# yjxiong/action-detection

Measured on NVIDIA H100. Metric: proposals/sec (9-seg BNInception SSN fwd+bwd), higher is better.
Workload: dtype f32 via split f16 operands (hi+lo, 3 wgmma MMAs per product) / f32 accumulate; f32 storage

## Files before the change

### action-detection_b200/csrc/common.cuh

```cuda
#pragma once
#include <cuda_fp16.h>
#include <cuda_runtime.h>
#include <stdint.h>

#include <atomic>
#include <string>

namespace ssnb {

struct View {
  void* base = nullptr;
  int H = 0, W = 0, C = 0, pitch = 0, coff = 0;
  long long lo_off = 0;
};

extern std::atomic<long long> g_launches;
void set_thread_error(const std::string& s);
const std::string& thread_error();

struct LaunchTag {
  int phase = 3;
  double flop = 0.0;
  const char* op = nullptr;
  int tiles = 0, block_n = 0;
};
extern thread_local bool t_timing;
extern thread_local LaunchTag t_tag;
void timing_mark(const char* what, cudaStream_t s);

#define SSNB_LAUNCH_CHECK(what)                                                       \
  do {                                                                                \
    ssnb::g_launches.fetch_add(1, std::memory_order_relaxed);                         \
    cudaError_t _e = cudaGetLastError();                                              \
    if (_e != cudaSuccess) {                                                          \
      ssnb::set_thread_error(std::string(what) + ": " + cudaGetErrorString(_e));      \
      return 2;                                                                       \
    }                                                                                 \
    if (ssnb::t_timing) ssnb::timing_mark(what, s);                                   \
  } while (0)

template <typename T> __device__ __forceinline__ float to_f(T v);
template <> __device__ __forceinline__ float to_f<float>(float v) { return v; }
template <> __device__ __forceinline__ float to_f<__half>(__half v) { return __half2float(v); }
template <typename T> __device__ __forceinline__ T from_f(float v);
template <> __device__ __forceinline__ float from_f<float>(float v) { return v; }
template <> __device__ __forceinline__ __half from_f<__half>(float v) { return __float2half_rn(v); }
__device__ __forceinline__ float relu(float v) { return v <= 0.f ? 0.f : v; }

constexpr float HALF_MAX = 65504.f;
__device__ __forceinline__ void split2(float a, float b, uint32_t& hi, uint32_t& lo) {
  const __half2 h = __floats2half2_rn(a, b);
  const float2 hf = __half22float2(h);
  const __half2 l = __floats2half2_rn(a - hf.x, b - hf.y);
  hi = *reinterpret_cast<const uint32_t*>(&h);
  lo = *reinterpret_cast<const uint32_t*>(&l);
}
__device__ __forceinline__ void store_planes4(__half* hi, long long lo_off, const float4& v) {
  uint2 h, l;
  split2(v.x, v.y, h.x, l.x);
  split2(v.z, v.w, h.y, l.y);
  *reinterpret_cast<uint2*>(hi) = h;
  *reinterpret_cast<uint2*>(reinterpret_cast<char*>(hi) + lo_off) = l;
}

struct ConvArgs {
  const void* src; int SH, SW, Csrc, src_pitch, src_coff;
  void* dst;       int DH, DW, Cdst, dst_pitch, dst_coff;
  const void* wgt;
  const float* bias;
  int F, kh, kw, stride, pad_h, pad_w;
  int relu, accumulate, dgrad;
};
struct WgradArgs {
  const void* dz; int OH, OW, Cout, dz_pitch, dz_coff;
  const void* x;  int IH, IW, Cin, x_pitch, x_coff;
  float* partial;
  int F, k, stride, pad, rows_per_split, splits;
};
template <typename T> int launch_conv(const ConvArgs& a, cudaStream_t s);
template <typename T> int launch_wgrad(const WgradArgs& a, cudaStream_t s);
int launch_wgrad_finalize(const float* partial, int splits, int taps, int Cout, int Cin, const float* mult,
                          float out_scale, float* dw_ref, int accumulate, cudaStream_t s, const float* bias_partial = nullptr,
                          float* db = nullptr, int* flag = nullptr,
                          const float* unscale = nullptr);

template <typename T> int launch_nchw_to_nhwc(const float* src, int F, int C, int H, int W, View dst, float scale, cudaStream_t s);
template <typename T> int launch_nhwc_to_nchw(View src, int F, float scale, float* dst, cudaStream_t s);
template <typename T> int launch_gpool_fwd(View src, int F, float* feat, cudaStream_t s);
template <typename T> int launch_gpool_bwd(const float* dfeat, float scale, const float* scale_dev, View ddst, int F, const void* y,
                                           cudaStream_t s);
constexpr int GRAD_EXP_TOP = 8, GRAD_EXP_MAX = 100;
int launch_grad_exponent(const float* dfeat, long long n, float grad_scale, int HW, float* gscale, int* flag, cudaStream_t s);

constexpr int PACK_MAX = 32;
constexpr int PACK_PER_THREAD = 4;
constexpr int PACK_TILE = 32, PACK_TILE_TAPS = 9;
inline int pack_ctas(int cout, int cin, int taps) {
  if (taps <= PACK_TILE_TAPS) return ((cout + PACK_TILE - 1) / PACK_TILE) * ((cin + PACK_TILE - 1) / PACK_TILE);
  const long long n = (long long)cout * cin * taps, per = 256LL * PACK_PER_THREAD;
  return (int)(((n > cout ? n : cout) + per - 1) / per);
}
struct PackEntry {
  const float *w, *b, *gamma, *beta, *mean, *var;
  void *wf, *wd; float *bias, *scale, *absmax;
  int cout, cin, taps, block0;
  int nofold, pad_[3];
  float* bias_b;
};
struct PackTable { int n, pad_; PackEntry e[PACK_MAX]; };
template <typename T> int launch_pack_all(const PackTable& t, int total_blocks, cudaStream_t s);
struct SplitEntry {
  const float *wf, *wd; __half *wf16, *wd16; long long plane_bytes, n; const float* absmax; float* inv_scale; int block0, pad_;
  __half *wd16_b, *wf16_b; long long b_plane_bytes; int b_pitch, cout;
};
struct SplitTable { int n, pad_; SplitEntry e[PACK_MAX]; };
int launch_split_all(const SplitTable& t, int total_blocks, cudaStream_t s);

constexpr int FIN_MAX = 36;
struct FinalizeEntry {
  const float* partial; const float* mult; float* dw; const float* bias_partial; float* db;
  int splits, taps, Cout, Cin, block0, pad_;
};
struct FinalizeTable { int n, total_blocks; int* flag; const float* unscale; FinalizeEntry e[FIN_MAX]; };
int launch_wgrad_finalize_all(const FinalizeTable& t, float out_scale, int accumulate, cudaStream_t s);

template <typename T> constexpr int VEC_WIDTH = 16 / (int)sizeof(T);
template <typename T>
int launch_maxpool_fwd_vec(View src, View dst, View dst_planes, int F, int k, int stride, int pad, uint8_t* argmax, cudaStream_t s);
template <typename T>
int launch_maxpool_bwd_vec(View dsrc, View ddst, int F, int k, int stride, int pad, const uint8_t* argmax, int accumulate, cudaStream_t s);
template <typename T> int launch_avgpool3_vec(View src, View dst, View dst_planes, int F, int accumulate, cudaStream_t s);
template <typename T>
int launch_mask_bias_vec(View dy, View y, View planes, float scale, int write_back, int* flag, int F, const float* mult, float out_scale,
                         const float* unscale, float* partial, int max_ctas, float* db, int accumulate, cudaStream_t s);
template <typename T>
int launch_pool_mask_bias_vec(View dz, View y, View dpool, View planes, float scale, int write_back, int* flag, int F, int k, int stride, int pad,
                              const uint8_t* argmax, const float* mult, float out_scale, const float* unscale, float* partial, int max_ctas,
                              float* db, int accumulate, cudaStream_t s);
int launch_split_view(View src_f32, int F, float scale, View planes, int* flag, cudaStream_t s);
int launch_planes_to_nchw(View planes, int F, float scale, float* dst, cudaStream_t s);
int launch_bn_train_fwd(View z, View y, View y_planes, int F, const float* gamma, const float* beta, float eps, float momentum, float* running_mean,
                        float* running_var, float* stat, float* partial, int max_ctas, cudaStream_t s);
int launch_bn_train_bwd(View z, View dy, View y, View dz, View dz_planes, float plane_scale, int* flag, int F, const float* gamma, float* stat,
                        float* partial, int max_ctas, float* dgamma, float* dbeta, const float* unscale, int accumulate, cudaStream_t s);
int launch_nhwc_to_s2d(View src, int F, __half* dst, long long lo_off, int Cs, cudaStream_t s);
int launch_nchw_to_s2d(const float* src, int F, int Cin, int H, int W, __half* dst, long long lo_off, int Cs, cudaStream_t s);
int launch_pack_conv1_s2d(const __half* wd, int Cout, int Cin, int Cs, __half* ws, cudaStream_t s);
int launch_wgrad_finalize_s2d(const float* partial, int splits, int Cout, int Cin, int Cs, const float* mult, float out_scale,
                              const float* unscale, float* dw_ref, int accumulate, cudaStream_t s);
int launch_upsample2_zero(View src, __half* dst, int H, int W, int F, cudaStream_t s);

}
```

### action-detection_b200/csrc/engine.cu

```cuda
#include <cstdio>
#include <cstdlib>
#include <algorithm>
#include <cstring>
#include <map>
#include <string>
#include <vector>

#include <cuda_profiler_api.h>

#include "../../include/ssnb.h"
#include "common.cuh"
#include "graph.cuh"
#include "umma_conv.cuh"

namespace ssnb {

std::atomic<long long> g_launches{0};
static thread_local std::string t_error;
void set_thread_error(const std::string& s) { t_error = s; }
const std::string& thread_error() { return t_error; }

thread_local bool t_timing = false;
thread_local LaunchTag t_tag;
struct TimingMark { const char* what; LaunchTag tag; std::string op; cudaEvent_t ev; };
static thread_local std::vector<TimingMark> t_marks;
static thread_local std::vector<cudaEvent_t> t_event_pool;
static thread_local std::string t_report;
static cudaEvent_t timing_event() {
  if (!t_event_pool.empty()) { cudaEvent_t e = t_event_pool.back(); t_event_pool.pop_back(); return e; }
  cudaEvent_t e = nullptr;
  cudaEventCreate(&e);
  return e;
}
void timing_mark(const char* what, cudaStream_t s) {
  TimingMark m{what, t_tag, t_tag.op ? t_tag.op : "", timing_event()};
  m.tag.op = nullptr;
  if (m.ev && cudaEventRecord(m.ev, s) == cudaSuccess) t_marks.push_back(m);
  else cudaGetLastError();
  t_tag.flop = 0.0; t_tag.op = nullptr; t_tag.tiles = 0; t_tag.block_n = 0;
}

static bool timing_close() {
  t_timing = false;
  if (t_marks.empty()) return false;
  if (cudaEventSynchronize(t_marks.back().ev) != cudaSuccess) { cudaGetLastError(); return false; }
  return true;
}

struct BlockSpec { const char* name; int c1, c3r, c3, cdr, cd1, cd2; int pool_max; int cproj; int stride; };
static const BlockSpec kBlocks[10] = {
    {"3a", 64, 64, 64, 64, 96, 96, 0, 32, 1},      {"3b", 64, 64, 96, 64, 96, 96, 0, 64, 1},
    {"3c", 0, 128, 160, 64, 96, 96, 1, 0, 2},      {"4a", 224, 64, 96, 96, 128, 128, 0, 128, 1},
    {"4b", 192, 96, 128, 96, 128, 128, 0, 128, 1}, {"4c", 160, 128, 160, 128, 160, 160, 0, 128, 1},
    {"4d", 96, 128, 192, 160, 192, 192, 0, 128, 1}, {"4e", 0, 128, 192, 192, 256, 256, 1, 0, 2},
    {"5a", 352, 192, 320, 160, 224, 224, 0, 128, 1}, {"5b", 352, 192, 320, 192, 224, 224, 1, 128, 1}};

static std::vector<Conv> conv_table(int in_ch) {
  std::vector<Conv> v;
  auto add = [&](const std::string& id, int cin, int cout, int k, int stride, int pad) { v.push_back({id, cin, cout, k, k, stride, pad, pad}); };
  add("conv1_7x7_s2", in_ch, 64, 7, 2, 3);
  add("conv2_3x3_reduce", 64, 64, 1, 1, 0);
  add("conv2_3x3", 64, 192, 3, 1, 1);
  int cx = 192;
  for (const BlockSpec& b : kBlocks) {
    std::string p = std::string("inception_") + b.name + "_";
    if (b.c1) add(p + "1x1", cx, b.c1, 1, 1, 0);
    add(p + "3x3_reduce", cx, b.c3r, 1, 1, 0);
    add(p + "3x3", b.c3r, b.c3, 3, b.stride, 1);
    add(p + "double_3x3_reduce", cx, b.cdr, 1, 1, 0);
    add(p + "double_3x3_1", b.cdr, b.cd1, 3, 1, 1);
    add(p + "double_3x3_2", b.cd1, b.cd2, 3, b.stride, 1);
    if (b.cproj) add(p + "pool_proj", cx, b.cproj, 1, 1, 0);
    cx = b.c1 + b.c3 + b.cd2 + (b.cproj ? b.cproj : cx);
  }
  return v;
}

struct Op : GraphOp {
  int grad_accumulate = 0;
  int wsplits = 1, wrows = 0;
  int tsplits = 1;
  size_t partial_off = 0, bias_partial_off = 0;
  UmmaConvPlan umma;
  UmmaConvPlan umma_dgrad;
  UmmaWgradPlan umma_wgrad;
  int pool_consumer = -1;
  bool folded_into_conv = false;
  bool dgrad_masks = false;
  bool bias_in_wgrad = false;
  bool dy_premasked = false;
  bool raw = false;
  int fuse_role = 0;
  int fuse_block = -1;
};
struct FusedBlock {
  int op1 = -1, op_r3 = -1, op_rd = -1;
  int c1 = 0, c3r = 0, cdr = 0, cx = 0;
  size_t w_fwd = 0, bias = 0, w_dg = 0;
  size_t w_fwd_plane = 0, w_dg_plane = 0, wmax = 0;
  UmmaConvPlan fwd, dgrad;
  bool enabled = false;
};

}

using namespace ssnb;

struct ssnb_engine : ssnb::Graph<ssnb::Op> {
  ssnb_config cfg;
  size_t up_plane = 0, s2d_plane = 0, s2d_w_plane = 0;
  int* tc_flag = nullptr;
  size_t tc_flag_off = 0;
  float* gscale = nullptr;
  bool bn1_train = false;
  const float *bn1_gamma = nullptr, *bn1_beta = nullptr; float *bn1_rmean = nullptr, *bn1_rvar = nullptr, *bn1_dgamma = nullptr, *bn1_dbeta = nullptr;
  float bn1_momentum = 0.1f, bn1_eps = 1e-5f;
  size_t bn_stat_off = 0, bn_partial_off = 0;
  std::vector<FusedBlock> fused;
  size_t ws_bytes = 0, partial_off = 0, partial_bytes = 0, bpartial_off = 0;
  size_t s2d_off = 0, s2d_w_off = 0, up_off = 0;
  bool fold_pools = true;
  bool s2d_ready = false;
  int Cs = 0;
  int conv1_tsplits = 128;
  bool weights_ready = false;
  std::vector<float*> dw, db;
  std::vector<int> pending_finalize;
  int grad_accumulate = 0;
  std::string error;
  long long launches0 = 0;
  UmmaContext umma_ctx;

  int fail(int code, const std::string& msg) { error = msg; return code; }
  const float* grad_scale_dev() const { return tensor_cores() ? gscale : nullptr; }
  const float* grad_unscale_dev() const { return tensor_cores() ? gscale + 1 : nullptr; }
  int nplanes() const { return exact_tc() ? 2 : 1; }
  const __half* w_fwd(const PackedConv& p) const { return (const __half*)(ws + (exact_tc() ? p.wd16 : p.wd)); }
  const __half* w_dgrad(const PackedConv& p) const { return (const __half*)(ws + (exact_tc() ? p.wf16 : p.wf)); }
  const UmmaTcOpts* tc_opts(UmmaTcOpts& t, size_t w_lo_off, void* out32, float alpha, size_t wmax) const {
    if (!exact_tc()) return nullptr;
    t.w_lo_off = (long long)w_lo_off; t.out32 = (float*)out32; t.alpha = alpha; t.alpha_dev = (const float*)(ws + wmax) + 1;
    return &t;
  }
};

namespace ssnb {

static bool profiled_op(const char* env, const std::string& id) {
  const char* e = getenv(env);
  if (!e || !*e) return false;
  const std::string list = std::string(",") + e + ",";
  return list.find("," + id + ",") != std::string::npos;
}
static bool env_on(const char* name) {
  const char* v = getenv(name);
  return v && v[0] == '1';
}
static int device_sms() {
  int dev = 0, sms = 0;
  if (cudaGetDevice(&dev) != cudaSuccess || cudaDeviceGetAttribute(&sms, cudaDevAttrMultiProcessorCount, dev) != cudaSuccess || sms <= 0) {
    cudaGetLastError();
    return 132;
  }
  return sms;
}

static void build_graph(ssnb_engine* e) {
  const int cin = e->cfg.in_channels;
  e->convs = conv_table(cin);
  int ci = 0;
  auto conv_op = [&](int in, int out) {
    const Conv& c = e->convs[ci];
    Op o; o.kind = OP_CONV; o.id = c.id; o.in = in; o.out = out; o.conv = ci;
    o.k = c.kh; o.stride = c.stride; o.pad = c.ph;
    e->ops.push_back(o);
    ++ci;
  };
  auto pool_op = [&](OpKind kind, const std::string& id, int in, int out, int k, int s, int p) {
    Op o; o.kind = kind; o.id = id; o.in = in; o.out = out; o.k = k; o.stride = s; o.pad = p;
    e->ops.push_back(o);
  };
  int x = e->whole("data", 224, 224, cin);
  int v;
  if (e->bn1_train) {
    const int raw = e->whole("conv1_7x7_s2_raw", 112, 112, 64); conv_op(x, raw); e->ops.back().raw = true;
    v = e->whole("conv1_7x7_s2_bn", 112, 112, 64);
    pool_op(OP_BN1, "conv1_7x7_s2_bn", raw, v, 0, 1, 0); x = v;
  } else {
    v = e->whole("conv1_7x7_s2_bn", 112, 112, 64); conv_op(x, v); x = v;
  }
  v = e->whole("pool1_3x3_s2", 56, 56, 64); pool_op(OP_MAXPOOL, "pool1_3x3_s2", x, v, 3, 2, 0); x = v;
  v = e->whole("conv2_3x3_reduce_bn", 56, 56, 64); conv_op(x, v); x = v;
  v = e->whole("conv2_3x3_bn", 56, 56, 192); conv_op(x, v); x = v;
  v = e->whole("pool2_3x3_s2", 28, 28, 192); pool_op(OP_MAXPOOL, "pool2_3x3_s2", x, v, 3, 2, 0); x = v;
  int H = 28, cx = 192;
  for (const BlockSpec& b : kBlocks) {
    const std::string p = std::string("inception_") + b.name + "_";
    const int OHW = (b.stride == 2) ? pool_out(H, 3, 2, 0) : H;
    const int ctot = b.c1 + b.c3 + b.cd2 + (b.cproj ? b.cproj : cx);
    const int cat = e->add_buffer(p + "output", OHW, OHW, ctot);
    const int red = e->add_buffer(p + "reduce", H, H, b.c3r + b.cdr);
    int off = 0;
    if (b.c1) { v = e->add_value(p + "1x1_bn", cat, off, b.c1); conv_op(x, v); off += b.c1; }
    int r3 = e->add_value(p + "3x3_reduce_bn", red, 0, b.c3r); conv_op(x, r3);
    v = e->add_value(p + "3x3_bn", cat, off, b.c3); conv_op(r3, v); off += b.c3;
    int rd = e->add_value(p + "double_3x3_reduce_bn", red, b.c3r, b.cdr); conv_op(x, rd);
    int d1 = e->whole(p + "double_3x3_1_bn", H, H, b.cd1); conv_op(rd, d1);
    v = e->add_value(p + "double_3x3_2_bn", cat, off, b.cd2); conv_op(d1, v); off += b.cd2;
    if (b.stride == 2) {
      v = e->add_value(p + "pool", cat, off, cx);
      pool_op(OP_MAXPOOL, p + "pool", x, v, 3, 2, 0);
    } else {
      int pl = e->whole(p + "pool", H, H, cx);
      pool_op(b.pool_max ? OP_MAXPOOL : OP_AVGPOOL, p + "pool", x, pl, 3, 1, 1);
      v = e->add_value(p + "pool_proj_bn", cat, off, b.cproj); conv_op(pl, v);
    }
    x = e->add_value(p + "output", cat, 0, ctot);
    H = OHW; cx = ctot;
  }
  Op g; g.kind = OP_GPOOL; g.id = "global_pool"; g.in = x; g.out = -1; g.k = 7;
  e->ops.push_back(g);
}

static void plan(ssnb_engine* e) {
  const size_t F = (size_t)e->F;
  size_t off = 0;
  e->tc_flag_off = off; off = align_up(off + 256, 1024);
  if (e->bn1_train) { e->bn_stat_off = off; off = align_up(off + 4 * 64 * 4, 1024); e->bn_partial_off = off; off = align_up(off + (size_t)1200 * 2 * 64 * 4, 1024); }
  off = e->plan_storage(off, e->cfg.training != 0, e->convs[0].cin, 16);
  size_t pmax = 0;
  if (e->cfg.training) {
    std::vector<char> written(e->vals.size(), 0);
    for (int i = (int)e->ops.size() - 1; i >= 0; --i) {
      Op& o = e->ops[i];
      o.grad_accumulate = written[o.in];
      written[o.in] = 1;
      if (o.kind == OP_CONV) {
        const Conv& c = e->convs[o.conv];
        const Buffer& ob = e->bufs[e->vals[o.out].buf];
        const long long M = (long long)F * ob.H * ob.W;
        const int taps = c.kh * c.kw;
        const bool flat = c.cin < 16;
        const long long tiles = (long long)((c.cout + 63) / 64) * (flat ? (taps * c.cin + 63) / 64 : ((c.cin + 63) / 64) * taps);
        long long splits = (592 + tiles - 1) / tiles;
        if (splits > 128) splits = 128;
        while (splits > 1 && M / splits < 256) --splits;
        long long rows = (M + splits - 1) / splits;
        rows = (rows + 15) / 16 * 16;
        splits = (M + rows - 1) / rows;
        o.wsplits = (int)splits; o.wrows = (int)rows;
        {
          const int chunks = (c.cin + 63) / 64, n_tiles = (chunks + 3) / 4, block_n = ((chunks + n_tiles - 1) / n_tiles) * 64;
          const int tpc = std::max(1, 4 / (block_n / 64));
          const int ctas = ((c.cout + 127) / 128) * n_tiles * ((taps + tpc - 1) / tpc);
          o.tsplits = std::max(o.wsplits, std::min(128, umma_wgrad_splits(ctas, umma_wgrad_ptiles(ob.W, ob.H, e->F), device_sms())));
        }
        if (e->tensor_cores()) splits = std::max<long long>(splits, o.tsplits);
        const size_t need = (size_t)splits * taps * c.cout * c.cin * 4;
        if (need > pmax) pmax = need;
      }
    }
  }
  if (e->tensor_cores()) {
    for (int i = 0; i < (int)e->ops.size(); ++i) {
      const Op& o = e->ops[i];
      if (o.kind != OP_CONV || o.k != 1) continue;
      const std::string& id = o.id;
      const std::string suf = "_3x3_reduce";
      if (id.size() < suf.size() || id.compare(id.size() - suf.size(), suf.size(), suf) != 0 || id.find("double") != std::string::npos) continue;
      const std::string pre = id.substr(0, id.size() - suf.size() + 1);
      FusedBlock fb; fb.op_r3 = i;
      for (int j = 0; j < (int)e->ops.size(); ++j) {
        if (e->ops[j].id == pre + "1x1") fb.op1 = j;
        if (e->ops[j].id == pre + "double_3x3_reduce") fb.op_rd = j;
      }
      if (fb.op_rd < 0) continue;
      fb.cx = e->convs[o.conv].cin; fb.c3r = e->convs[o.conv].cout; fb.cdr = e->convs[e->ops[fb.op_rd].conv].cout;
      fb.c1 = fb.op1 >= 0 ? e->convs[e->ops[fb.op1].conv].cout : 0;
      const int n = fb.c1 + fb.c3r + fb.cdr, kf = (fb.c1 + 63) / 64 * 64 + fb.c3r + fb.cdr;
      fb.w_fwd_plane = align_up((size_t)n * fb.cx * 2, 1024); fb.w_dg_plane = align_up((size_t)fb.cx * kf * 2, 1024);
      if (e->exact_tc()) fb.w_fwd_plane = fb.w_dg_plane = std::max(fb.w_fwd_plane, fb.w_dg_plane);
      fb.w_fwd = off; off += e->nplanes() * fb.w_fwd_plane;
      fb.bias = off; off = align_up(off + (size_t)n * 4, 256);
      fb.w_dg = off; off += e->nplanes() * fb.w_dg_plane;
      if (e->exact_tc()) {
        if (e->fused.size() >= 16) continue;
        fb.wmax = e->wmax_off + (e->convs.size() + e->fused.size()) * 8;
        for (int j : {fb.op1, fb.op_r3, fb.op_rd}) if (j >= 0) e->packed[e->ops[j].conv].wmax = fb.wmax;
      }
      e->fused.push_back(fb);
    }
  }
  if (e->tensor_cores()) {
    for (int i = 0; i < (int)e->ops.size(); ++i) {
      Op& po = e->ops[i];
      if (po.kind != OP_MAXPOOL || po.k != 3 || po.stride != 2 || po.pad != 0) continue;
      int producer = -1, consumers = 0;
      for (int j = 0; j < (int)e->ops.size(); ++j) {
        if (e->ops[j].out == po.in && e->ops[j].kind == OP_CONV) producer = j;
        if (e->ops[j].in == po.in) ++consumers;
      }
      if (producer >= 0 && consumers == 1 && e->vals[po.in].C % (e->fast() ? VEC_WIDTH<__half> : VEC_WIDTH<float>) == 0) { e->ops[producer].pool_consumer = i; po.folded_into_conv = true; }
    }
    auto operand_region = [&](size_t bytes, size_t& plane) {
      const size_t at = off;
      if (e->exact_tc()) { plane = align_up(bytes, 1024); off += 2 * plane; }
      else off = align_up(off + bytes, 1024);
      return at;
    };
    e->Cs = (4 * e->cfg.in_channels + 7) / 8 * 8;
    {
      const int chunks = (4 * e->Cs + 63) / 64, n_tiles = (chunks + 3) / 4, block_n = ((chunks + n_tiles - 1) / n_tiles) * 64;
      const int tpc = std::min(4, std::max(1, 4 / (block_n / 64)));
      const int ptiles = umma_wgrad_ptiles(112, 112, e->F);
      if ((ptiles + UMMA_WGRAD_MAX_PTILES - 1) / UMMA_WGRAD_MAX_PTILES > 128)
        e->conv1_tsplits = umma_wgrad_splits(n_tiles * ((4 + tpc - 1) / tpc), ptiles, device_sms());
    }
    e->s2d_off = operand_region(F * 112 * 112 * 4 * e->Cs * 2, e->s2d_plane);
    e->s2d_w_off = operand_region((size_t)16 * 64 * e->Cs * 2, e->s2d_w_plane);
    if (e->cfg.training) {
      size_t up = 0;
      for (const Op& o : e->ops)
        if (o.kind == OP_CONV && o.stride == 2 && o.conv != 0) {
          const Buffer& ib = e->bufs[e->vals[o.in].buf];
          up = std::max(up, F * ib.H * ib.W * (size_t)e->convs[o.conv].cout * 2);
        }
      e->up_off = operand_region(up, e->up_plane);
      pmax = std::max(pmax, (size_t)e->conv1_tsplits * 16 * 64 * e->Cs * 4);
    }
  }
  e->partial_off = off; e->partial_bytes = pmax; off = align_up(off + pmax, 1024);
  if (e->cfg.training)
    for (Op& o : e->ops)
      if (o.kind == OP_CONV) {
        const Conv& c = e->convs[o.conv];
        const int nsplit = e->tensor_cores() ? std::max(o.wsplits, o.tsplits) : o.wsplits;
        size_t need = (size_t)nsplit * c.kh * c.kw * c.cout * c.cin * 4;
        if (o.conv == 0 && e->tensor_cores()) need = std::max(need, (size_t)e->conv1_tsplits * 16 * 64 * e->Cs * 4);
        o.partial_off = off; off = align_up(off + need, 1024);
        o.bias_partial_off = off; off = align_up(off + (size_t)std::max(nsplit, 128) * c.cout * 4, 256);
      }
  e->bpartial_off = off; off = align_up(off + (size_t)1024 * 512 * 4, 1024);
  e->ws_bytes = off;
}

#define DISPATCH(e, call_f, call_h) ((e)->fast() ? (call_h) : (call_f))

static inline void tag_next(int phase, double flop, const char* op = nullptr) { t_tag.phase = phase; t_tag.flop = flop; t_tag.op = op; }
static thread_local std::string t_fused_name;
static const char* fused_name(const ssnb_engine* e, const FusedBlock& fb) {
  if (!t_timing) return nullptr;
  t_fused_name.clear();
  for (int j : {fb.op1, fb.op_r3, fb.op_rd})
    if (j >= 0) t_fused_name += (t_fused_name.empty() ? "" : "+") + e->ops[j].id;
  return t_fused_name.c_str();
}

static int run_fwd(ssnb_engine* e, const Op& o, float* feat, int n, cudaStream_t s) {
  tag_next(0, 0.0);
  if (o.kind == OP_CONV && o.umma.enabled) {
    if (o.conv == 0 && !e->s2d_ready) {
      const View in = e->view(o.in, false);
      __half* s2d = (__half*)(e->ws + e->s2d_off);
      if (int rc = launch_nhwc_to_s2d(in, n, s2d, (long long)e->s2d_plane, e->Cs, s)) return rc;
    }
    tag_next(0, e->conv_flops(o, n), o.id.c_str());
    return umma_conv_launch(e->umma_ctx, o.umma, s, false, n);
  }
  if (o.kind == OP_BN1) {
    if (!e->bn1_gamma || !e->bn1_beta) { set_thread_error("bn1_train engine: call ssnb_set_bn1 first"); return SSNB_ESTATE; }
    return launch_bn_train_fwd(e->view(o.in, false), e->view(o.out, false), e->exact_tc() ? e->planes(o.out, false) : View(), e->F, e->bn1_gamma,
                               e->bn1_beta, e->bn1_eps, e->bn1_momentum, e->bn1_rmean, e->bn1_rvar, (float*)(e->ws + e->bn_stat_off),
                               (float*)(e->ws + e->bn_partial_off), 1200, s);
  }
  if (o.kind == OP_MAXPOOL || o.kind == OP_AVGPOOL) return e->pool_fwd(o, n, s);
  if (o.kind == OP_GPOOL) {
    if (!feat) return e->fail(SSNB_EINVAL, "global_pool needs the feat output pointer");
    return e->gpool_fwd(o, n, feat, s);
  }
  if (int rc = e->simt_conv_fwd(o, o.raw ? 0 : 1, n, s)) return rc;
  if (!e->exact_tc() || !e->bufs[e->vals[o.out].buf].plane) return 0;
  return launch_split_view(e->view(o.out), n, 1.0f, e->planes(o.out), nullptr, s);
}

static int simt_wgrad(ssnb_engine* e, const Op& o, cudaStream_t s) {
  const Conv& c = e->convs[o.conv];
  const View x = e->view(o.in, false), dz = e->view(o.out, true);
  float* partial = (float*)(e->ws + o.partial_off);
  WgradArgs w;
  w.dz = dz.base; w.OH = dz.H; w.OW = dz.W; w.Cout = dz.C; w.dz_pitch = dz.pitch; w.dz_coff = dz.coff;
  w.x = x.base; w.IH = x.H; w.IW = x.W; w.Cin = x.C; w.x_pitch = x.pitch; w.x_coff = x.coff;
  w.partial = partial; w.F = e->F; w.k = c.kh; w.stride = c.stride; w.pad = c.ph;
  w.rows_per_split = o.wrows; w.splits = o.wsplits;
  tag_next(2, e->conv_flops(o, e->F), o.id.c_str());
  if (int rc = DISPATCH(e, launch_wgrad<float>(w, s), launch_wgrad<__half>(w, s))) return rc;
  const float out_scale = e->fast() ? 1.0f / e->cfg.grad_scale : 1.0f;
  return launch_wgrad_finalize(partial, o.wsplits, c.kh * c.kw, c.cout, c.cin, (const float*)(e->ws + e->packed[o.conv].scale), out_scale,
                               e->dw[o.conv], e->grad_accumulate, s, nullptr, nullptr, nullptr, e->grad_unscale_dev());
}
static int simt_dgrad(ssnb_engine* e, const Op& o, cudaStream_t s) {
  const Conv& c = e->convs[o.conv];
  const View dz = e->view(o.out, true), dx = e->view(o.in, true);
  ConvArgs a;
  a.src = dz.base; a.SH = dz.H; a.SW = dz.W; a.Csrc = dz.C; a.src_pitch = dz.pitch; a.src_coff = dz.coff;
  a.dst = dx.base; a.DH = dx.H; a.DW = dx.W; a.Cdst = dx.C; a.dst_pitch = dx.pitch; a.dst_coff = dx.coff;
  a.wgt = e->ws + e->packed[o.conv].wd; a.bias = nullptr;
  a.F = e->F; a.kh = a.kw = c.kh; a.stride = c.stride; a.pad_h = a.pad_w = c.ph; a.relu = 0; a.accumulate = o.grad_accumulate; a.dgrad = 1;
  tag_next(1, e->conv_flops(o, e->F), o.id.c_str());
  return DISPATCH(e, launch_conv<float>(a, s), launch_conv<__half>(a, s));
}

static int run_bwd(ssnb_engine* e, const Op& o, const float* dfeat, cudaStream_t s, bool skip_dgrad = false, bool full = false) {
  const int F = e->F;
  const float gs = e->fast() ? e->cfg.grad_scale : 1.0f;
  int rc = 0;
  tag_next(3, 0.0);
  if (o.kind == OP_GPOOL) {
    if (!dfeat) return e->fail(SSNB_EINVAL, "global_pool backward needs dfeat");
    const View din = e->view(o.in, true);
    const void* ym = (full && e->fold_pools && o.dgrad_masks) ? e->view(o.in, false).base : nullptr;
    const float* gsd = e->grad_scale_dev();
    return DISPATCH(e, launch_gpool_bwd<float>(dfeat, gs, gsd, din, F, ym, s), launch_gpool_bwd<__half>(dfeat, gs, gsd, din, F, ym, s));
  }
  if (o.kind == OP_BN1) {
    return launch_bn_train_bwd(e->view(o.in, false), e->view(o.out, true), e->view(o.out, false), e->view(o.in, true),
                               e->exact_tc() ? e->planes(o.in, true) : View(), e->cfg.grad_scale, e->tc_flag, F, e->bn1_gamma, (float*)(e->ws + e->bn_stat_off),
                               (float*)(e->ws + e->bn_partial_off), 1200, e->bn1_dgamma, e->bn1_dbeta, e->grad_unscale_dev(), e->grad_accumulate, s);
  }
  if (o.kind == OP_MAXPOOL) {
    if (full && e->fold_pools && o.folded_into_conv) return 0;
    const View din = e->view(o.in, true), dout = e->view(o.out, true);
    const uint8_t* am = (const uint8_t*)(e->ws + o.argmax_off);
    return DISPATCH(e, launch_maxpool_bwd_vec<float>(din, dout, F, o.k, o.stride, o.pad, am, o.grad_accumulate, s),
                    launch_maxpool_bwd_vec<__half>(din, dout, F, o.k, o.stride, o.pad, am, o.grad_accumulate, s));
  }
  if (o.kind == OP_AVGPOOL) {
    const View din = e->view(o.in, true), dout = e->view(o.out, true);
    return DISPATCH(e, launch_avgpool3_vec<float>(dout, din, View(), F, o.grad_accumulate, s),
                    launch_avgpool3_vec<__half>(dout, din, View(), F, o.grad_accumulate, s));
  }
  const Conv& c = e->convs[o.conv];
  const View x = e->view(o.in, false), y = e->view(o.out, false), dy = e->view(o.out, true);
  const float* scale = (const float*)(e->ws + e->packed[o.conv].scale);
  float* bpartial = (float*)(e->ws + e->bpartial_off);
  float* dbp = (e->db.size() && e->db[o.conv]) ? e->db[o.conv] : nullptr;
  const bool want_w = e->dw.size() && e->dw[o.conv];
  const bool want_x = e->vals[o.in].name != "data" && !skip_dgrad;
  const float gst = e->cfg.grad_scale;
  const float* us = e->grad_unscale_dev();
  const bool tc_w = want_w && o.umma_wgrad.enabled, tc_x = want_x && o.umma_dgrad.enabled;
  const bool pre = full && e->fold_pools && o.dy_premasked;
  const bool bias_w = pre && o.bias_in_wgrad && dbp && tc_w;
  const Op* pool = (full && e->fold_pools && o.pool_consumer >= 0) ? &e->ops[o.pool_consumer] : nullptr;
  const int max_ctas = (1024 * 512 - 64) / y.C;
  const View dpool = pool ? e->view(pool->out, true) : View();
  const uint8_t* pam = pool ? (const uint8_t*)(e->ws + pool->argmax_off) : nullptr;
  if (e->fast()) {
    if (pool) rc = launch_pool_mask_bias_vec<__half>(dy, y, dpool, View(), 1.0f, 1, nullptr, F, pool->k, pool->stride, pool->pad, pam,
                                                    scale, 1.0f / gst, us, bpartial, max_ctas, dbp, e->grad_accumulate, s);
    else if (!bias_w) rc = launch_mask_bias_vec<__half>(dy, pre ? View() : y, View(), 1.0f, 1, nullptr, F, scale, 1.0f / gst, us, bpartial, max_ctas, dbp,
                                                       e->grad_accumulate, s);
  } else {
    const bool need_f32 = (want_w && !tc_w) || (want_x && !tc_x);
    const View pl = (tc_w || tc_x) ? e->planes(o.out, true) : View();
    if (o.raw) {
      if (dbp) rc = launch_mask_bias_vec<float>(dy, View(), View(), gst, 0, nullptr, F, scale, 1.0f, us, bpartial, max_ctas, dbp, e->grad_accumulate, s);
    } else if (pre) {
      if (!bias_w && dbp) rc = launch_mask_bias_vec<float>(dy, y, View(), gst, 0, nullptr, F, scale, 1.0f, us, bpartial, max_ctas, dbp, e->grad_accumulate, s);
    } else if (pool) {
      rc = launch_pool_mask_bias_vec<float>(dy, y, dpool, pl, gst, need_f32 ? 1 : 0, e->tc_flag, F, pool->k, pool->stride, pool->pad, pam,
                                            scale, 1.0f, us, bpartial, max_ctas, dbp, e->grad_accumulate, s);
    } else {
      rc = launch_mask_bias_vec<float>(dy, y, pl, gst, (need_f32 || !full) ? 1 : 0, e->tc_flag, F, scale, 1.0f, us, bpartial, max_ctas, dbp,
                                       e->grad_accumulate, s);
    }
  }
  if (rc) return rc;
  if (tc_x && c.stride == 2 && o.conv != 0) {
    View dz = e->operand(o.out, true);
    for (int p = 0; p < e->nplanes(); ++p, dz.base = (char*)dz.base + dz.lo_off)
      if ((rc = launch_upsample2_zero(dz, (__half*)(e->ws + e->up_off + p * e->up_plane), x.H, x.W, F, s))) return rc;
  }
  if (tc_w) {
    float* partial = (float*)(e->ws + o.partial_off);
    float* bp = bias_w ? (float*)(e->ws + o.bias_partial_off) : nullptr;
    tag_next(2, e->conv_flops(o, F), o.id.c_str());
    if ((rc = umma_wgrad_launch(e->umma_ctx, o.umma_wgrad, s, bp))) return rc;
    if (full && o.conv != 0) e->pending_finalize.push_back((int)(&o - e->ops.data()));
    else if (o.conv == 0) rc = launch_wgrad_finalize_s2d(partial, o.umma_wgrad.p.splits, c.cout, c.cin, e->Cs, scale, 1.0f / gst, us, e->dw[o.conv],
                                                         e->grad_accumulate, s);
    else rc = launch_wgrad_finalize(partial, o.umma_wgrad.p.splits, c.kh * c.kw, c.cout, c.cin, scale, 1.0f / gst, e->dw[o.conv], e->grad_accumulate, s,
                                    nullptr, nullptr, e->tc_flag, us);
    if (rc) return rc;
  } else if (want_w && (rc = simt_wgrad(e, o, s))) return rc;
  if (tc_x) {
    tag_next(1, e->conv_flops(o, F), o.id.c_str());
    return umma_conv_launch(e->umma_ctx, o.umma_dgrad, s, full && e->fold_pools && o.dgrad_masks);
  }
  return want_x ? simt_dgrad(e, o, s) : 0;
}

int engine_tail_view(ssnb_handle h, View* v, int* F, int* fp16) {
  if (!h->ws || !h->weights_ready) return h->fail(SSNB_ESTATE, "workspace/weights not set");
  *v = h->view(h->ops.back().in, false);
  *F = h->F; *fp16 = h->fast() ? 1 : 0;
  return 0;
}

}

extern "C" {

const char* ssnb_version(void) { return "libssn_b200 0.3 (sm_90a)"; }

const char* ssnb_last_error(ssnb_handle h) { return h ? h->error.c_str() : ssnb::thread_error().c_str(); }

int ssnb_num_convs(void) { return 69; }

int ssnb_conv_info(int idx, int in_channels, char* name, int name_cap, int* cin, int* cout, int* k, int* stride, int* pad) {
  std::vector<Conv> t = conv_table(in_channels);
  if (idx < 0 || idx >= (int)t.size()) { set_thread_error("ssnb_conv_info: index out of range"); return SSNB_EINVAL; }
  if (name && name_cap > 0) { snprintf(name, name_cap, "%s", t[idx].id.c_str()); }
  if (cin) *cin = t[idx].cin; if (cout) *cout = t[idx].cout; if (k) *k = t[idx].kh;
  if (stride) *stride = t[idx].stride; if (pad) *pad = t[idx].ph;
  return SSNB_OK;
}

int ssnb_create(const ssnb_config* cfg, ssnb_handle* out) {
  if (!cfg || !out) { set_thread_error("ssnb_create: null argument"); return SSNB_EINVAL; }
  if (cfg->frames <= 0 || cfg->in_channels <= 0 || cfg->in_channels > 64) { set_thread_error("ssnb_create: bad frames/in_channels"); return SSNB_EINVAL; }
  if (cfg->precision != SSNB_EXACT_FP32 && cfg->precision != SSNB_FAST_FP16 && cfg->precision != SSNB_EXACT_TC) { set_thread_error("ssnb_create: unknown precision"); return SSNB_EINVAL; }
  ssnb_engine* e = new ssnb_engine();
  e->cfg = *cfg;
  if (!(e->cfg.grad_scale > 0.f)) e->cfg.grad_scale = 1.0f;
  e->F = cfg->frames;
  e->precision = cfg->precision;
  e->bn1_train = cfg->bn1_train != 0;
  if (e->bn1_train && e->fast()) { delete e; set_thread_error("ssnb_create: bn1_train (bn_mode='partial') needs EXACT_FP32 or EXACT_TC"); return SSNB_ENOSUPPORT; }
  e->esz = e->fast() ? 2 : 4;
  build_graph(e);
  if ((int)e->convs.size() != 69) { delete e; set_thread_error("internal: conv table size"); return SSNB_ESTATE; }
  umma_context_init(e->umma_ctx);
  plan(e);
  e->launches0 = g_launches.load();
  *out = e;
  return SSNB_OK;
}

int ssnb_destroy(ssnb_handle h) {
  if (!h) return SSNB_OK;
  umma_context_destroy(h->umma_ctx);
  delete h;
  return SSNB_OK;
}

size_t ssnb_workspace_bytes(ssnb_handle h) { return h ? h->ws_bytes : 0; }

int ssnb_set_workspace(ssnb_handle h, void* dev_ptr, size_t bytes) {
  if (!h) return SSNB_EINVAL;
  if (!dev_ptr || bytes < h->ws_bytes) return h->fail(SSNB_EINVAL, "workspace too small");
  if (((uintptr_t)dev_ptr) % 1024) return h->fail(SSNB_EINVAL, "workspace must be 1024-byte aligned");
  h->ws = (char*)dev_ptr;
  h->weights_ready = false;
  if (cudaMemset(h->ws + h->bpartial_off, 0, 256) != cudaSuccess) { cudaGetLastError();  }
  h->tc_flag = (int*)(h->ws + h->tc_flag_off);
  if (cudaMemset(h->tc_flag, 0, 256) != cudaSuccess) cudaGetLastError();
  h->gscale = (float*)(h->ws + h->tc_flag_off + 16);
  const float one[2] = {1.0f, 1.0f};
  if (cudaMemcpy(h->gscale, one, sizeof one, cudaMemcpyHostToDevice) != cudaSuccess) cudaGetLastError();
  const bool training = h->cfg.training != 0;
  const bool use_tc = h->tensor_cores() && !env_on("SSNB_DISABLE_UMMA");
  const bool use_wgrad = use_tc && training && !env_on("SSNB_DISABLE_UMMA_WGRAD");
  const bool fuse = !env_on("SSNB_DISABLE_FUSION");
  const float gs = h->cfg.grad_scale;
  for (Op& o : h->ops) {
    o.umma.enabled = o.umma_dgrad.enabled = o.umma_wgrad.enabled = false;
    o.fuse_role = 0; o.fuse_block = -1; o.dgrad_masks = o.dy_premasked = o.bias_in_wgrad = false;
  }
  for (FusedBlock& fb : h->fused) fb.enabled = false;
  h->fold_pools = fuse && (h->fast() || (use_tc && training));
  auto tc_gate = [&](UmmaConvPlan& p) {
    if (h->exact_tc() && !p.p.tc_ok) p.enabled = false;
    return p.enabled;
  };
  for (Op& o : h->ops) {
    if (o.kind != OP_CONV || !use_tc) continue;
    const Conv& c = h->convs[o.conv];
    const PackedConv& pk = h->packed[o.conv];
    UmmaTcOpts tf, tg;
    int rc = 0;
    if (o.conv == 0) {
      const int Ck = 4 * h->Cs;
      View xs; xs.base = h->ws + h->s2d_off; xs.H = 112; xs.W = 112; xs.C = Ck; xs.pitch = Ck; xs.coff = 0; xs.lo_off = (long long)h->s2d_plane;
      int dy[4], dx[4];
      for (int t = 0; t < 4; ++t) { dy[t] = t - 2; dx[t] = 0; }
      rc = umma_conv_bind_taps(h->umma_ctx, o.umma, xs, h->operand(o.out, false), h->F, Ck, c.cout, 4, dy, dx, (const __half*)(h->ws + h->s2d_w_off),
                               (const float*)(h->ws + pk.bias), o.raw ? 0 : 1, h->tc_opts(tf, h->s2d_w_plane, h->view(o.out, false).base, 1.0f, pk.wmax));
      if (rc) return h->fail(rc, "conv1 bind: " + ssnb::thread_error());
      tc_gate(o.umma);
      if (use_wgrad && (rc = umma_wgrad_bind_taps(h->umma_ctx, o.umma_wgrad, h->operand(o.out, true), xs, h->F, Ck, c.cout, 4, dy, dx,
                                                  (float*)(h->ws + o.partial_off), h->conv1_tsplits)))
        return h->fail(rc, "conv1 wgrad bind: " + ssnb::thread_error());
      continue;
    }
    if (c.cin % 8 != 0 || c.kh * c.kw > UMMA_MAX_TAPS) continue;
    rc = umma_conv_bind_fwd(h->umma_ctx, o.umma, h->operand(o.in, false), h->operand(o.out, false), h->F, c.cin, c.cout, c.kh, c.ph,
                            c.stride, h->w_fwd(pk), (const float*)(h->ws + pk.bias), h->tc_opts(tf, pk.wplane, h->view(o.out, false).base, 1.0f, pk.wmax));
    if (rc) return h->fail(rc, "bind_fwd(" + c.id + "): " + ssnb::thread_error());
    if (!training) continue;
    const View in = h->view(o.in, false);
    View dz = h->operand(o.out, true);
    if (c.stride == 2) { dz.base = h->ws + h->up_off; dz.H = in.H; dz.W = in.W; dz.C = c.cout; dz.pitch = c.cout; dz.coff = 0; dz.lo_off = (long long)h->up_plane; }
    View dx = h->view(o.in, true);
    const UmmaTcOpts* og = h->tc_opts(tg, pk.wplane, dx.base, 1.0f / gs, pk.wmax);
    if (og) dx.base = nullptr;
    rc = umma_conv_bind_dgrad(h->umma_ctx, o.umma_dgrad, dz, dx, h->F, c.cin, c.cout, c.kh, c.ph, h->w_dgrad(pk), o.grad_accumulate, og);
    if (rc) return h->fail(rc, "bind_dgrad(" + c.id + "): " + ssnb::thread_error());
    tc_gate(o.umma_dgrad);
    if (use_wgrad && (rc = umma_wgrad_bind(h->umma_ctx, o.umma_wgrad, h->operand(o.out, true), h->operand(o.in, false), h->F, c.cin, c.cout,
                                           c.kh, c.ph, (float*)(h->ws + o.partial_off), o.tsplits, c.stride)))
      return h->fail(rc, "wgrad_bind(" + c.id + "): " + ssnb::thread_error());
  }
  for (size_t bi = 0; bi < h->fused.size() && use_tc && fuse; ++bi) {
    FusedBlock& fb = h->fused[bi];
    const Op& o3 = h->ops[fb.op_r3]; const Op& od = h->ops[fb.op_rd];
    if (!o3.umma.enabled || !od.umma.enabled) continue;
    const int nr = fb.c3r + fb.cdr;
    const View x = h->operand(o3.in, false);
    View red = h->operand(o3.out, false); red.C = nr;
    UmmaTcOpts tf, tg;
    int rc;
    if (fb.op1 >= 0) {
      const int v1 = h->ops[fb.op1].out;
      const UmmaTcOpts* of = h->tc_opts(tf, fb.w_fwd_plane, h->view(v1, false).base, 1.0f, fb.wmax);
      tf.out32_2 = (float*)h->view(o3.out, false).base;
      rc = umma_conv_bind_fused_fwd(h->umma_ctx, fb.fwd, x, h->operand(v1, false), red, h->F, fb.cx, fb.c1, nr, (const __half*)(h->ws + fb.w_fwd),
                                    (const float*)(h->ws + fb.bias), of);
    } else {
      rc = umma_conv_bind_fwd(h->umma_ctx, fb.fwd, x, red, h->F, fb.cx, nr, 1, 0, 1, (const __half*)(h->ws + fb.w_fwd), (const float*)(h->ws + fb.bias),
                              h->tc_opts(tf, fb.w_fwd_plane, h->view(o3.out, false).base, 1.0f, fb.wmax));
    }
    if (rc) return h->fail(rc, "fused fwd bind(" + o3.id + "): " + ssnb::thread_error());
    if (!tc_gate(fb.fwd)) continue;
    if (training) {
      View dred = h->operand(o3.out, true); dred.C = nr;
      const View d1 = fb.op1 >= 0 ? h->operand(h->ops[fb.op1].out, true) : dred;
      View dx = h->view(o3.in, true);
      const UmmaTcOpts* og = h->tc_opts(tg, fb.w_dg_plane, dx.base, 1.0f / gs, fb.wmax);
      if (og) dx.base = nullptr;
      rc = umma_conv_bind_fused_dgrad(h->umma_ctx, fb.dgrad, d1, dred, dx, h->F, fb.cx, fb.c1, nr, (const __half*)(h->ws + fb.w_dg), od.grad_accumulate, og);
      if (rc) return h->fail(rc, "fused dgrad bind(" + o3.id + "): " + ssnb::thread_error());
      if (!tc_gate(fb.dgrad)) continue;
      if (h->exact_tc() && cudaMemset(h->ws + fb.w_dg, 0, 2 * fb.w_dg_plane) != cudaSuccess) cudaGetLastError();
    }
    fb.enabled = true;
    const int leader = fb.op1 >= 0 ? fb.op1 : fb.op_r3;
    for (int j : {fb.op1, fb.op_r3, fb.op_rd})
      if (j >= 0) { h->ops[j].fuse_block = (int)bi; h->ops[j].fuse_role = (j == leader) ? 1 : 2; }
  }
  if (use_tc && training && fuse) {
    std::vector<int> first_consumer(h->vals.size(), -1);
    for (int i = 0; i < (int)h->ops.size(); ++i)
      if (first_consumer[h->ops[i].in] < 0) first_consumer[h->ops[i].in] = i;
    for (size_t v = 0; v < h->vals.size(); ++v) {
      const int fc = first_consumer[v];
      if (fc < 0 || h->vals[v].name == "data") continue;
      if (h->exact_tc() && !h->bufs[h->vals[v].buf].plane) continue;
      bool conv_made = false;
      for (const Op& q : h->ops) conv_made = conv_made || (q.kind == OP_CONV && h->vals[q.out].buf == h->vals[v].buf);
      if (!conv_made) continue;
      Op& c = h->ops[fc];
      UmmaConvPlan* dg = nullptr;
      if (c.kind == OP_CONV && c.fuse_role == 1 && h->fused[c.fuse_block].enabled) dg = &h->fused[c.fuse_block].dgrad;
      else if (c.kind == OP_CONV && c.fuse_role == 0 && c.umma_dgrad.enabled) dg = &c.umma_dgrad;
      if (dg) {
        c.dgrad_masks = true;
        if (h->exact_tc()) {
          if (int rc = umma_conv_set_mask_tc(h->umma_ctx, *dg, h->view((int)v, false), h->planes((int)v, true), gs, h->tc_flag))
            return h->fail(rc, "mask bind(" + h->vals[v].name + "): " + ssnb::thread_error());
        } else {
          umma_conv_set_mask(*dg, h->view((int)v, false));
        }
      } else if (c.kind == OP_GPOOL && h->fast()) {
        c.dgrad_masks = true;
      }
    }
    for (Op& o : h->ops) {
      if (o.kind != OP_CONV) continue;
      int w = o.out;
      if (first_consumer[w] < 0) {
        const Value& ov = h->vals[o.out];
        for (size_t v = 0; v < h->vals.size(); ++v)
          if (h->vals[v].buf == ov.buf && h->vals[v].coff == 0 && h->vals[v].C == h->bufs[ov.buf].C && first_consumer[v] >= 0) { w = (int)v; break; }
      }
      if (first_consumer[w] >= 0 && h->ops[first_consumer[w]].dgrad_masks) o.dy_premasked = true;
      o.bias_in_wgrad = o.dy_premasked && o.conv != 0 && o.umma_wgrad.enabled;
    }
  }
  return SSNB_OK;
}

int ssnb_pack_weights(ssnb_handle h, const float* const* w, const float* const* b, const float* const* gamma,
                      const float* const* beta, const float* const* mean, const float* const* var, void* stream) {
  if (!h || !h->ws) return h ? h->fail(SSNB_ESTATE, "set_workspace first") : SSNB_EINVAL;
  cudaStream_t s = (cudaStream_t)stream;
  struct Member { int block = -1, row = 0, col = 0; };
  std::vector<Member> member(h->convs.size());
  for (size_t bi = 0; bi < h->fused.size(); ++bi) {
    const FusedBlock& fb = h->fused[bi];
    if (!fb.enabled) continue;
    const int k1p = (fb.c1 + 63) / 64 * 64;
    int row = 0, col = 0;
    for (int j : {fb.op1, fb.op_r3, fb.op_rd}) {
      if (j < 0) continue;
      const int ci = h->ops[j].conv;
      member[ci].block = (int)bi; member[ci].row = row; member[ci].col = col;
      row += h->convs[ci].cout;
      col += (j == fb.op1) ? k1p : h->convs[ci].cout;
    }
  }
  auto adjust = [&](size_t i, PackEntry& q, SplitEntry* e) {
    q.nofold = (h->bn1_train && i == 0) ? 1 : 0;
    const Member& mb = member[i];
    if (!h->exact_tc() || mb.block < 0) return;
    const FusedBlock& fb = h->fused[mb.block];
    q.bias_b = (float*)(h->ws + fb.bias) + mb.row;
    const int kf = (fb.c1 + 63) / 64 * 64 + fb.c3r + fb.cdr;
    e->wd16_b = (__half*)(h->ws + fb.w_fwd) + (size_t)mb.row * fb.cx;
    e->wf16_b = (__half*)(h->ws + fb.w_dg) + mb.col;
    e->b_pitch = kf;
    e->b_plane_bytes = (long long)std::max(fb.w_fwd_plane, fb.w_dg_plane);
  };
  if (int rc = h->pack_weights(w, b, gamma, beta, mean, var, h->convs[0].cin, adjust, "pack_weights", s)) return h->fail(rc, ssnb::thread_error());
  if (h->ops.size() && h->ops[0].umma.enabled) {
    const PackedConv& p = h->packed[0];
    for (int pl = 0; pl < h->nplanes(); ++pl) {
      int rc = launch_pack_conv1_s2d((const __half*)((const char*)h->w_fwd(p) + pl * p.wplane), h->convs[0].cout, h->convs[0].cin, h->Cs,
                                     (__half*)(h->ws + h->s2d_w_off + pl * h->s2d_w_plane), s);
      if (rc) return h->fail(rc, "pack conv1 s2d: " + ssnb::thread_error());
    }
  }
  for (FusedBlock& fb : h->fused) {
    if (!fb.enabled || !h->fast()) continue;
    const int k1p = (fb.c1 + 63) / 64 * 64, kf = k1p + fb.c3r + fb.cdr;
    __half* wfwd = (__half*)(h->ws + fb.w_fwd); float* bias = (float*)(h->ws + fb.bias); __half* wdg = (__half*)(h->ws + fb.w_dg);
    if (cudaMemsetAsync(wdg, 0, (size_t)fb.cx * kf * 2, s) != cudaSuccess) return h->fail(SSNB_ECUDA, "fused pack: memset");
    int row = 0, col = 0;
    for (int j : {fb.op1, fb.op_r3, fb.op_rd}) {
      if (j < 0) { continue; }
      const int ci = h->ops[j].conv, co = h->convs[ci].cout;
      cudaError_t e1 = cudaMemcpyAsync(wfwd + (size_t)row * fb.cx, h->ws + h->packed[ci].wd, (size_t)co * fb.cx * 2, cudaMemcpyDeviceToDevice, s);
      cudaError_t e2 = cudaMemcpyAsync(bias + row, h->ws + h->packed[ci].bias, (size_t)co * 4, cudaMemcpyDeviceToDevice, s);
      cudaError_t e3 = cudaMemcpy2DAsync(wdg + col, (size_t)kf * 2, h->ws + h->packed[ci].wf, (size_t)co * 2, (size_t)co * 2, fb.cx,
                                         cudaMemcpyDeviceToDevice, s);
      if (e1 != cudaSuccess || e2 != cudaSuccess || e3 != cudaSuccess) return h->fail(SSNB_ECUDA, "fused pack: copy failed");
      row += co;
      col += (j == fb.op1) ? k1p : co;
    }
  }
  h->weights_ready = true;
  return SSNB_OK;
}

int ssnb_set_bn1(ssnb_handle h, const float* gamma, const float* beta, float* running_mean, float* running_var, float* dgamma, float* dbeta,
                 float momentum, float eps) {
  if (!h) return SSNB_EINVAL;
  if (!h->bn1_train) return h->fail(SSNB_ESTATE, "engine created without bn1_train");
  if (!gamma || !beta) return h->fail(SSNB_EINVAL, "set_bn1: gamma / beta are required");
  h->bn1_gamma = gamma; h->bn1_beta = beta; h->bn1_rmean = running_mean; h->bn1_rvar = running_var; h->bn1_dgamma = dgamma; h->bn1_dbeta = dbeta;
  h->bn1_momentum = momentum; h->bn1_eps = eps;
  return SSNB_OK;
}

static int backbone_fwd(ssnb_handle h, const float* input_nchw, int n, float* feat, cudaStream_t s) {
  const View d = h->view(h->val_by_name["data"], false);
  int rc;
  h->s2d_ready = h->tensor_cores() && h->ops[0].umma.enabled;
  if (h->s2d_ready) rc = launch_nchw_to_s2d(input_nchw, n, d.C, d.H, d.W, (__half*)(h->ws + h->s2d_off), (long long)h->s2d_plane, h->Cs, s);
  else rc = h->value_write(h->val_by_name["data"], false, input_nchw, 1.0f, n, s);
  if (rc) { h->s2d_ready = false; return h->fail(rc, "input layout: " + ssnb::thread_error()); }
  for (size_t i = 0; i < h->ops.size(); ++i) {
    const Op& o = h->ops[i];
    if (o.fuse_role == 2) continue;
    const bool prof = profiled_op("SSNB_PROFILE_FWD_OPS", o.id);
    if (prof) cudaProfilerStart();
    int r;
    if (o.fuse_role == 1) {
      const FusedBlock& fb = h->fused[o.fuse_block];
      double fl = 0.0;
      for (int j : {fb.op1, fb.op_r3, fb.op_rd}) if (j >= 0) fl += h->conv_flops(h->ops[j], n);
      tag_next(0, fl, fused_name(h, fb));
      r = umma_conv_launch(h->umma_ctx, fb.fwd, s, false, n);
    } else r = run_fwd(h, o, feat, n, s);
    if (prof) cudaProfilerStop();
    if (r) { h->s2d_ready = false; return h->fail(r, "fwd " + o.id + ": " + ssnb::thread_error()); }
  }
  h->s2d_ready = false;
  return SSNB_OK;
}

int ssnb_backbone_fwd(ssnb_handle h, const float* input_nchw, float* feat, void* stream) {
  if (!h || !input_nchw || !feat) return h ? h->fail(SSNB_EINVAL, "null argument") : SSNB_EINVAL;
  if (!h->ws || !h->weights_ready) return h->fail(SSNB_ESTATE, "workspace/weights not set");
  return backbone_fwd(h, input_nchw, h->F, feat, (cudaStream_t)stream);
}

int ssnb_backbone_fwd_frames(ssnb_handle h, const float* input_nchw, int frames, float* feat, void* stream) {
  if (!h || !input_nchw || !feat) return h ? h->fail(SSNB_EINVAL, "null argument") : SSNB_EINVAL;
  if (frames < 1 || frames > h->F) return h->fail(SSNB_EINVAL, "backbone_fwd_frames: frames must be in 1 .. " + std::to_string(h->F));
  if (h->cfg.training) return h->fail(SSNB_ESTATE, "backbone_fwd_frames: runs forward-only engines (training = 0)");
  if (h->bn1_train) return h->fail(SSNB_ENOSUPPORT, "backbone_fwd_frames: bn1_train engines run their planned frame count only");
  if (!h->ws || !h->weights_ready) return h->fail(SSNB_ESTATE, "workspace/weights not set");
  return backbone_fwd(h, input_nchw, frames, feat, (cudaStream_t)stream);
}

int ssnb_bind_grads(ssnb_handle h, float* const* dw, float* const* db) {
  if (!h) return SSNB_EINVAL;
  h->dw.assign(h->convs.size(), nullptr); h->db.assign(h->convs.size(), nullptr);
  for (size_t i = 0; i < h->convs.size(); ++i) { if (dw) h->dw[i] = dw[i]; if (db) h->db[i] = db[i]; }
  return SSNB_OK;
}

int ssnb_backbone_bwd(ssnb_handle h, const float* dfeat, float* const* dw, float* const* db, void* stream) {
  return ssnb_backbone_bwd_range(h, dfeat, dw, db, -1, 0, stream);
}

int ssnb_backbone_bwd_range(ssnb_handle h, const float* dfeat, float* const* dw, float* const* db, int op_hi, int op_lo, void* stream) {
  if (!h || (!dfeat && (op_hi < 0 || op_hi >= (int)h->ops.size() - 1))) return h ? h->fail(SSNB_EINVAL, "null argument") : SSNB_EINVAL;
  if (!h->cfg.training) return h->fail(SSNB_ESTATE, "engine created without training=1");
  if (!h->ws || !h->weights_ready) return h->fail(SSNB_ESTATE, "workspace/weights not set");
  ssnb_bind_grads(h, dw, db);
  h->pending_finalize.clear();
  cudaStream_t s = (cudaStream_t)stream;
  auto run_range = [&](int hi, int lo) -> int {
    for (int i = hi; i >= lo; --i) {
      const Op& o = h->ops[i];
      const bool prof = profiled_op("SSNB_PROFILE_BWD_OPS", o.id);
      if (prof) cudaProfilerStart();
      int rc = run_bwd(h, o, dfeat, s, o.fuse_role != 0, true);
      if (!rc && o.fuse_role == 1) {
        const FusedBlock& fb = h->fused[o.fuse_block];
        double fl = 0.0;
        for (int j : {fb.op1, fb.op_r3, fb.op_rd}) if (j >= 0) fl += h->conv_flops(h->ops[j], h->F);
        tag_next(1, fl, fused_name(h, fb));
        rc = umma_conv_launch(h->umma_ctx, fb.dgrad, s, h->fold_pools && o.dgrad_masks);
      }
      if (prof) cudaProfilerStop();
      if (rc) return h->fail(rc, "bwd " + o.id + ": " + ssnb::thread_error());
    }
    return 0;
  };
  auto finalize = [&]() -> int {
    const float gs = h->tensor_cores() ? h->cfg.grad_scale : 1.0f;
    FinalizeTable t; t.n = 0; t.total_blocks = 0; t.flag = h->tc_flag; t.unscale = h->grad_unscale_dev();
    auto flush = [&]() -> int { int rc = launch_wgrad_finalize_all(t, 1.0f / gs, h->grad_accumulate, s); t.n = 0; t.total_blocks = 0; return rc; };
    for (int oi : h->pending_finalize) {
      const Op& o = h->ops[oi];
      const Conv& c = h->convs[o.conv];
      FinalizeEntry& q = t.e[t.n];
      q.partial = (const float*)(h->ws + o.partial_off); q.mult = (const float*)(h->ws + h->packed[o.conv].scale); q.dw = h->dw[o.conv];
      const bool bias_w = o.dy_premasked && o.bias_in_wgrad && h->db.size() && h->db[o.conv];
      q.bias_partial = bias_w ? (const float*)(h->ws + o.bias_partial_off) : nullptr; q.db = bias_w ? h->db[o.conv] : nullptr;
      q.splits = o.umma_wgrad.p.splits; q.taps = c.kh * c.kw; q.Cout = c.cout; q.Cin = c.cin; q.block0 = t.total_blocks; q.pad_ = 0;
      t.total_blocks += (int)(((long long)q.taps * q.Cout * q.Cin + 255) / 256);
      if (++t.n == FIN_MAX) if (int rc = flush()) { h->pending_finalize.clear(); return h->fail(rc, "finalize: " + ssnb::thread_error()); }
    }
    h->pending_finalize.clear();
    if (int rc = flush()) return h->fail(rc, "finalize: " + ssnb::thread_error());
    return 0;
  };
  const int last = (int)h->ops.size() - 1;
  if (op_hi < 0 || op_hi > last) op_hi = last;
  if (op_lo < 0 || op_lo > op_hi) return h->fail(SSNB_EINVAL, "backbone_bwd_range: bad op range");
  if (op_hi == last && h->tensor_cores()) {
    if (int rc = launch_grad_exponent(dfeat, (long long)h->F * h->vals[h->ops[last].in].C, h->cfg.grad_scale,
                                      h->bufs[h->vals[h->ops[last].in].buf].H * h->bufs[h->vals[h->ops[last].in].buf].W, h->gscale, h->tc_flag, s))
      return h->fail(rc, "gradient exponent: " + ssnb::thread_error());
  }
  if (int rc = run_range(op_hi, op_lo)) return rc;
  return finalize();
}

int ssnb_set_grad_accumulate(ssnb_handle h, int accumulate) {
  if (!h) return SSNB_EINVAL;
  h->grad_accumulate = accumulate ? 1 : 0;
  return SSNB_OK;
}

int ssnb_num_ops(ssnb_handle h) { return h ? (int)h->ops.size() : 0; }

int ssnb_op_info(ssnb_handle h, int op, char* kind, int kind_cap, char* in_name, int in_cap, char* out_name, int out_cap) {
  if (!h || op < 0 || op >= (int)h->ops.size()) return SSNB_EINVAL;
  const Op& o = h->ops[op];
  if (kind) snprintf(kind, kind_cap, "%s", kOpKindName[o.kind]);
  if (in_name) snprintf(in_name, in_cap, "%s", h->vals[o.in].name.c_str());
  if (out_name) snprintf(out_name, out_cap, "%s", o.out >= 0 ? h->vals[o.out].name.c_str() : "feat");
  return SSNB_OK;
}

int ssnb_value_shape(ssnb_handle h, const char* name, int* c, int* hh, int* ww) {
  if (!h || !name) return SSNB_EINVAL;
  const int v = h->value_of(name);
  if (v < 0) return h->fail(SSNB_EINVAL, std::string("unknown value ") + name);
  const View w = h->view(v, false);
  if (c) *c = w.C; if (hh) *hh = w.H; if (ww) *ww = w.W;
  return SSNB_OK;
}

static float host_gscale(ssnb_handle h, int which, cudaStream_t s) {
  float v = 1.0f;
  if (!h->tensor_cores() || cudaMemcpyAsync(&v, h->gscale + which, sizeof v, cudaMemcpyDeviceToHost, s) != cudaSuccess ||
      cudaStreamSynchronize(s) != cudaSuccess) { cudaGetLastError(); return 1.0f; }
  return v;
}

int ssnb_value_write(ssnb_handle h, const char* name, int grad, const float* src_nchw, void* stream) {
  if (!h || !name || !src_nchw || !h->ws) return SSNB_EINVAL;
  const int v = h->value_of(name);
  if (v < 0) return h->fail(SSNB_EINVAL, std::string("unknown value ") + name);
  if (grad && !h->cfg.training) return h->fail(SSNB_ESTATE, "no gradient buffers");
  const float sc = grad ? (h->fast() ? h->cfg.grad_scale : 1.0f) * host_gscale(h, 0, (cudaStream_t)stream) : 1.0f;
  const int rc = h->value_write(v, grad != 0, src_nchw, sc, h->F, (cudaStream_t)stream);
  return rc ? h->fail(rc, ssnb::thread_error()) : SSNB_OK;
}

int ssnb_value_read(ssnb_handle h, const char* name, int grad, float* dst_nchw, void* stream) {
  if (!h || !name || !dst_nchw || !h->ws) return SSNB_EINVAL;
  const int v = h->value_of(name);
  if (v < 0) return h->fail(SSNB_EINVAL, std::string("unknown value ") + name);
  if ((grad & 1) && !h->cfg.training) return h->fail(SSNB_ESTATE, "no gradient buffers");
  if (grad & 2) {
    if (!h->exact_tc() || !h->bufs[h->vals[v].buf].plane) return h->fail(SSNB_ESTATE, "value has no operand planes");
    const float sc = (grad & 1) ? host_gscale(h, 1, (cudaStream_t)stream) / h->cfg.grad_scale : 1.0f;
    const int rc = h->planes_read(v, (grad & 1) != 0, sc, dst_nchw, (cudaStream_t)stream);
    return rc ? h->fail(rc, ssnb::thread_error()) : SSNB_OK;
  }
  const float sc = grad ? host_gscale(h, 1, (cudaStream_t)stream) / (h->fast() ? h->cfg.grad_scale : 1.0f) : 1.0f;
  const int rc = h->value_read(v, grad != 0, sc, dst_nchw, (cudaStream_t)stream);
  return rc ? h->fail(rc, ssnb::thread_error()) : SSNB_OK;
}

int ssnb_run_op(ssnb_handle h, int op, int backward, void* stream) {
  if (!h || op < 0 || op >= (int)h->ops.size()) return SSNB_EINVAL;
  if (!h->ws || !h->weights_ready) return h->fail(SSNB_ESTATE, "workspace/weights not set");
  const Op& o = h->ops[op];
  if (o.kind == OP_GPOOL) return h->fail(SSNB_ENOSUPPORT, "run_op: global_pool runs through backbone_fwd/bwd");
  int rc = backward ? run_bwd(h, o, nullptr, (cudaStream_t)stream) : run_fwd(h, o, nullptr, h->F, (cudaStream_t)stream);
  return rc ? h->fail(rc, o.id + ": " + ssnb::thread_error()) : SSNB_OK;
}

int ssnb_grad_overflow(ssnb_handle h, int clear) {
  if (!h) return -1;
  if (!h->tc_flag) return 0;
  int v = 0;
  if (cudaMemcpy(&v, h->tc_flag, sizeof(int), cudaMemcpyDeviceToHost) != cudaSuccess) { cudaGetLastError(); return -1; }
  if (v && clear) cudaMemset(h->tc_flag, 0, sizeof(int));
  return v ? 1 : 0;
}

int ssnb_timing_begin(void* stream) {
  for (TimingMark& m : ssnb::t_marks) ssnb::t_event_pool.push_back(m.ev);
  ssnb::t_marks.clear();
  ssnb::t_tag = LaunchTag();
  ssnb::t_timing = true;
  ssnb::timing_mark("(begin)", (cudaStream_t)stream);
  return SSNB_OK;
}

const char* ssnb_timing_report(void) {
  ssnb::t_report.clear();
  if (!ssnb::timing_close()) return ssnb::t_report.c_str();
  struct Agg { int n = 0; double ms = 0, flop = 0; };
  std::map<std::pair<std::string, int>, Agg> agg;
  for (size_t i = 1; i < ssnb::t_marks.size(); ++i) {
    float ms = 0.f;
    if (cudaEventElapsedTime(&ms, ssnb::t_marks[i - 1].ev, ssnb::t_marks[i].ev) != cudaSuccess) { cudaGetLastError(); continue; }
    Agg& a = agg[{ssnb::t_marks[i].what, ssnb::t_marks[i].tag.phase}];
    a.n += 1; a.ms += ms; a.flop += ssnb::t_marks[i].tag.flop;
  }
  char line[256];
  for (const auto& kv : agg) {
    snprintf(line, sizeof line, "%s\t%d\t%d\t%.6f\t%.0f\n", kv.first.first.c_str(), kv.first.second, kv.second.n, kv.second.ms, kv.second.flop);
    ssnb::t_report += line;
  }
  return ssnb::t_report.c_str();
}

const char* ssnb_timing_launches(void) {
  ssnb::t_report.clear();
  if (!ssnb::timing_close()) return ssnb::t_report.c_str();
  char line[512];
  for (size_t i = 1; i < ssnb::t_marks.size(); ++i) {
    const ssnb::TimingMark& m = ssnb::t_marks[i];
    float ms = 0.f;
    if (cudaEventElapsedTime(&ms, ssnb::t_marks[i - 1].ev, m.ev) != cudaSuccess) { cudaGetLastError(); continue; }
    snprintf(line, sizeof line, "%s\t%d\t%s\t%.6f\t%.0f\t%d\t%d\n", m.what, m.tag.phase, m.op.empty() ? "-" : m.op.c_str(), ms, m.tag.flop,
             m.tag.tiles, m.tag.block_n);
    ssnb::t_report += line;
  }
  return ssnb::t_report.c_str();
}

int64_t ssnb_launch_count(ssnb_handle h) { return h ? (int64_t)(g_launches.load() - h->launches0) : 0; }
int64_t ssnb_global_launch_count(void) { return (int64_t)g_launches.load(); }

}
```

### action-detection_b200/csrc/s2d_glue.cu

```cuda
#include "common.cuh"

#include <type_traits>

namespace ssnb {
namespace {

template <typename T>
__global__ void nhwc_to_s2d_kernel(const T* __restrict__ src, int F, int H, int W, int Cin, int spitch, int scoff,
                                   __half* __restrict__ dst, long long lo_off, int Cs) {
  const int H2 = H / 2, W2 = W / 2, Ck = 4 * Cs;
  const long long total = (long long)F * H2 * W2 * Ck;
  const long long i = (long long)blockIdx.x * blockDim.x + threadIdx.x;
  if (i >= total) return;
  const int ch = (int)(i % Ck);
  const long long p = i / Ck;
  const int x2 = (int)(p % W2), y2 = (int)((p / W2) % H2);
  const long long f = p / ((long long)W2 * H2);
  const int ds = ch / Cs, q = ch % Cs;
  T v = 0.f;
  const int xs = x2 + ds - 2;
  if (q < 4 * Cin && xs >= 0 && xs < W2) {
    const int ab = q / Cin, c = q % Cin;
    v = src[((f * H + 2 * y2 + ab / 2) * W + 2 * xs + ab % 2) * spitch + scoff + c];
  }
  if constexpr (std::is_same_v<T, float>) {
    const __half h = __float2half_rn(v);
    dst[i] = h;
    *reinterpret_cast<__half*>(reinterpret_cast<char*>(dst + i) + lo_off) = __float2half_rn(v - __half2float(h));
  } else {
    dst[i] = v;
  }
}

__global__ void pack_conv1_s2d_kernel(const __half* __restrict__ wd, int Cout, int Cin, int Cs, __half* __restrict__ ws) {
  const int Ck = 4 * Cs;
  const long long total = (long long)4 * Cout * Ck;
  const long long i = (long long)blockIdx.x * blockDim.x + threadIdx.x;
  if (i >= total) return;
  const int ch = (int)(i % Ck);
  const int co = (int)((i / Ck) % Cout);
  const int dr = (int)(i / ((long long)Ck * Cout));
  const int ds = ch / Cs, q = ch % Cs;
  __half v = __float2half_rn(0.f);
  if (q < 4 * Cin) {
    const int ab = q / Cin, c = q % Cin;
    const int r = 2 * dr + ab / 2 - 1, s = 2 * ds + ab % 2 - 1;
    if (r >= 0 && r < 7 && s >= 0 && s < 7) v = wd[((long long)(r * 7 + s) * Cout + co) * Cin + c];
  }
  ws[i] = v;
}

__global__ void wgrad_finalize_s2d_kernel(const float* __restrict__ partial, int splits, int Cout, int Cin, int Cs,
                                          const float* __restrict__ mult, float out_scale, const float* __restrict__ unscale,
                                          float* __restrict__ dw, int accumulate) {
  const int Ck = 4 * Cs;
  const long long total = (long long)Cout * Cin * 49;
  const long long i = (long long)blockIdx.x * blockDim.x + threadIdx.x;
  if (i >= total) return;
  const int s = (int)(i % 7), r = (int)((i / 7) % 7);
  const int c = (int)((i / 49) % Cin), co = (int)(i / (49LL * Cin));
  const int dr = (r + 1) / 2, a = (r + 1) % 2, ds = (s + 1) / 2, b = (s + 1) % 2;
  const int ch = ds * Cs + (a * 2 + b) * Cin + c;
  float acc = 0.f;
  for (int sp = 0; sp < splits; ++sp) acc += partial[(((long long)sp * 4 + dr) * Cout + co) * Ck + ch];
  if (unscale) out_scale *= __ldg(unscale);
  dw[i] = (accumulate ? dw[i] : 0.f) + acc * mult[co] * out_scale;
}

template <int CS, int CIN, bool LO>
__global__ void nchw_to_s2d_kernel(const float* __restrict__ src, int F, int Cin_rt, int H, int W, __half* __restrict__ dst,
                                   long long lo_off) {
  const int Cin = CIN ? CIN : Cin_rt;
  const int H2 = H / 2, W2 = W / 2;
  const long long i = (long long)blockIdx.x * blockDim.x + threadIdx.x;
  if (i >= (long long)F * H2 * W2 * 4) return;
  const unsigned iu = (unsigned)i;
  const int ds = (int)(iu & 3u);
  const unsigned pu = iu >> 2;
  const int x2 = (int)(pu % (unsigned)W2), y2 = (int)((pu / (unsigned)W2) % (unsigned)H2);
  const long long p = pu;
  const long long f = pu / (unsigned)(W2 * H2);
  __align__(16) __half vh[CS];
  __align__(16) __half vl[LO ? CS : 1];
#pragma unroll
  for (int c = 0; c < CS; ++c) {
    vh[c] = __float2half_rn(0.f);
    if constexpr (LO) vl[c] = __float2half_rn(0.f);
  }
  const int xs = x2 + ds - 2;
  if (xs >= 0 && xs < W2) {
#pragma unroll
    for (int c = 0; c < Cin; ++c) {
      const float* pl = src + ((f * Cin + c) * H + 2 * y2) * (long long)W + 2 * xs;
      const float2 r0 = __ldg(reinterpret_cast<const float2*>(pl));
      const float2 r1 = __ldg(reinterpret_cast<const float2*>(pl + W));
      const float q[4] = {r0.x, r0.y, r1.x, r1.y};
#pragma unroll
      for (int ab = 0; ab < 4; ++ab) {
        const __half h = __float2half_rn(q[ab]);
        vh[ab * Cin + c] = h;
        if constexpr (LO) vl[ab * Cin + c] = __float2half_rn(q[ab] - __half2float(h));
      }
    }
  }
  __half* o = dst + p * (4 * CS) + ds * CS;
  uint4* oh = reinterpret_cast<uint4*>(o);
  uint4* ol = reinterpret_cast<uint4*>(reinterpret_cast<char*>(o) + lo_off);
#pragma unroll
  for (int q = 0; q < CS / 8; ++q) {
    oh[q] = reinterpret_cast<const uint4*>(vh)[q];
    if constexpr (LO) ol[q] = reinterpret_cast<const uint4*>(vl)[q];
  }
}

__global__ void upsample2_zero_kernel(const __half* __restrict__ src, int OH, int OW, int C, int spitch, int scoff,
                                      __half* __restrict__ dst, int H, int W, int F) {
  const int G = C / 8;
  const long long total = (long long)F * H * W * G;
  const long long i = (long long)blockIdx.x * blockDim.x + threadIdx.x;
  if (i >= total) return;
  const unsigned iu = (unsigned)i;
  const int g = (int)(iu % (unsigned)G);
  const unsigned pu = iu / (unsigned)G;
  const int x = (int)(pu % (unsigned)W), y = (int)((pu / (unsigned)W) % (unsigned)H);
  const long long p = pu;
  const long long f = pu / (unsigned)(W * H);
  uint4 v = make_uint4(0u, 0u, 0u, 0u);
  if (!(x & 1) && !(y & 1) && y / 2 < OH && x / 2 < OW)
    v = __ldg(reinterpret_cast<const uint4*>(src + ((f * OH + y / 2) * OW + x / 2) * spitch + scoff + g * 8));
  *reinterpret_cast<uint4*>(dst + p * C + g * 8) = v;
}

}

int launch_nhwc_to_s2d(View src, int F, __half* dst, long long lo_off, int Cs, cudaStream_t s) {
  const long long n = (long long)F * (src.H / 2) * (src.W / 2) * 4 * Cs;
  const unsigned g = (unsigned)((n + 255) / 256);
  if (lo_off) nhwc_to_s2d_kernel<float><<<g, 256, 0, s>>>((const float*)src.base, F, src.H, src.W, src.C, src.pitch, src.coff, dst, lo_off, Cs);
  else nhwc_to_s2d_kernel<__half><<<g, 256, 0, s>>>((const __half*)src.base, F, src.H, src.W, src.C, src.pitch, src.coff, dst, lo_off, Cs);
  SSNB_LAUNCH_CHECK("nhwc_to_s2d_kernel");
  return 0;
}
template <bool LO>
static int nchw_to_s2d(const float* src, int F, int Cin, int H, int W, __half* dst, long long lo_off, int Cs, cudaStream_t s) {
  const long long n = (long long)F * (H / 2) * (W / 2) * 4;
  const unsigned g = (unsigned)((n + 255) / 256);
  if (Cs == 16 && Cin == 3) nchw_to_s2d_kernel<16, 3, LO><<<g, 256, 0, s>>>(src, F, Cin, H, W, dst, lo_off);
  else if (Cs == 40 && Cin == 10) nchw_to_s2d_kernel<40, 10, LO><<<g, 256, 0, s>>>(src, F, Cin, H, W, dst, lo_off);
  else if (Cs == 16) nchw_to_s2d_kernel<16, 0, LO><<<g, 256, 0, s>>>(src, F, Cin, H, W, dst, lo_off);
  else if (Cs == 40) nchw_to_s2d_kernel<40, 0, LO><<<g, 256, 0, s>>>(src, F, Cin, H, W, dst, lo_off);
  else { set_thread_error("nchw_to_s2d: unsupported channel count (RGB 3 or Flow 10)"); return 1; }
  SSNB_LAUNCH_CHECK("nchw_to_s2d_kernel");
  return 0;
}
int launch_nchw_to_s2d(const float* src, int F, int Cin, int H, int W, __half* dst, long long lo_off, int Cs, cudaStream_t s) {
  return lo_off ? nchw_to_s2d<true>(src, F, Cin, H, W, dst, lo_off, Cs, s) : nchw_to_s2d<false>(src, F, Cin, H, W, dst, lo_off, Cs, s);
}
int launch_pack_conv1_s2d(const __half* wd, int Cout, int Cin, int Cs, __half* ws, cudaStream_t s) {
  const long long n = 16LL * Cout * Cs;
  pack_conv1_s2d_kernel<<<(unsigned)((n + 255) / 256), 256, 0, s>>>(wd, Cout, Cin, Cs, ws);
  SSNB_LAUNCH_CHECK("pack_conv1_s2d_kernel");
  return 0;
}
int launch_wgrad_finalize_s2d(const float* partial, int splits, int Cout, int Cin, int Cs, const float* mult, float out_scale,
                              const float* unscale, float* dw_ref, int accumulate, cudaStream_t s) {
  const long long n = (long long)Cout * Cin * 49;
  wgrad_finalize_s2d_kernel<<<(unsigned)((n + 255) / 256), 256, 0, s>>>(partial, splits, Cout, Cin, Cs, mult, out_scale, unscale, dw_ref, accumulate);
  SSNB_LAUNCH_CHECK("wgrad_finalize_s2d_kernel");
  return 0;
}
int launch_upsample2_zero(View src, __half* dst, int H, int W, int F, cudaStream_t s) {
  const long long n = (long long)F * H * W * (src.C / 8);
  upsample2_zero_kernel<<<(unsigned)((n + 255) / 256), 256, 0, s>>>((const __half*)src.base, src.H, src.W, src.C, src.pitch, src.coff, dst, H, W, F);
  SSNB_LAUNCH_CHECK("upsample2_zero_kernel");
  return 0;
}

}
```

### action-detection_b200/csrc/umma_conv.cu

```cuda
#include <cstdio>
#include <cstdlib>
#include <cstring>
#include <algorithm>

#include "umma_conv.cuh"
#include "umma_dev.cuh"

namespace ssnb {

namespace {

using namespace umma;
constexpr int MAX_STAGES = 8;
constexpr int PIPE_BYTES = 192 * 1024;
constexpr int A_BYTES = BLOCK_M * BLOCK_K * 2;
constexpr int NUM_THREADS = 384;
constexpr int N_STEP = 16;
constexpr int MAX_BLOCK_N = 128;
constexpr int EPI_COLS = 16;
constexpr int EPI_F32_BYTES = BLOCK_M * EPI_COLS * 4;
constexpr int EPI_F16_BYTES = BLOCK_M * EPI_COLS * 2;
constexpr int EPI_BYTES = EPI_F32_BYTES + 2 * EPI_F16_BYTES;
constexpr int BAR_BYTES = 256;
constexpr int SMEM_BYTES = PIPE_BYTES + 2 * EPI_BYTES + BAR_BYTES + 1024 ;
constexpr int ORDER_BAR = 1;
constexpr int EPI_BAR = 3;
static_assert(SMEM_BYTES <= 227 * 1024, "shared memory per block");

struct TileCoord { int w0, h0, f0, n0; };
__device__ __forceinline__ TileCoord decode_tile(const UmmaConvParams& p, int tile) {
  TileCoord t;
  const int nt = tile % p.n_tiles;
  int m = tile / p.n_tiles;
  t.n0 = nt * p.block_n;
  t.w0 = (m % p.tiles_w) * p.bw; m /= p.tiles_w;
  t.h0 = (m % p.tiles_h) * p.bh; m /= p.tiles_h;
  t.f0 = m * p.bf;
  return t;
}

__device__ __forceinline__ uint32_t sw64_off(int r, int c) { return r * 64 + ((((c >> 2) ^ (r >> 1)) & 3) << 4) + (c & 3) * 4; }
__device__ __forceinline__ uint32_t sw32_off(int r, int c) { return r * 32 + ((((c >> 3) ^ (r >> 2)) & 1) << 4) + (c & 7) * 2; }

__device__ __forceinline__ uint32_t h2_bits(__half2 h) { return *reinterpret_cast<const uint32_t*>(&h); }

template <int BN, int NK>
__device__ __forceinline__ void mma_k(float* d0, float* d1, uint32_t sa, uint32_t sb) {
#pragma unroll
  for (int k = 0; k < NK; ++k) {
    const uint64_t bdesc = make_desc_sw128(sb + k * MMA_K * 2);
    wgmma<BN, 0, 0>(d0, make_desc_sw128(sa + k * MMA_K * 2), bdesc);
    wgmma<BN, 0, 0>(d1, make_desc_sw128(sa + 64 * 128 + k * MMA_K * 2), bdesc);
  }
}

template <int BN, int NK>
__device__ __forceinline__ void mma_stage(float* d0, float* d1, uint32_t sa, uint32_t sb, uint32_t b_bytes, bool split) {
  if (split) {
    mma_k<BN, NK>(d0, d1, sa + A_BYTES, sb);
    mma_k<BN, NK>(d0, d1, sa, sb + b_bytes);
  }
  mma_k<BN, NK>(d0, d1, sa, sb);
}

__device__ __forceinline__ void ring_advance(uint32_t& stage, uint32_t& phase, int n, int stages) {
  const uint32_t s = stage + (uint32_t)n;
  phase ^= (s / (uint32_t)stages) & 1u;
  stage = s % (uint32_t)stages;
}

template <int BN, bool DIRECT>
__device__ __forceinline__ void
umma_conv_body(const CUtensorMap& tmap_a, const CUtensorMap& tmap_a2, const CUtensorMap& tmap_b, const CUtensorMap& tmap_a_lo,
               const CUtensorMap& tmap_a2_lo, const CUtensorMap& tmap_b_lo, const CUtensorMap& tmap_o, const CUtensorMap& tmap_o_hi,
               const CUtensorMap& tmap_o_lo, const CUtensorMap& tmap_o2, const CUtensorMap& tmap_o2_hi, const CUtensorMap& tmap_o2_lo,
               const UmmaConvParams& p) {
  extern __shared__ uint8_t smem_raw[];
  uint8_t* smem = reinterpret_cast<uint8_t*>((reinterpret_cast<uintptr_t>(smem_raw) + 1023) & ~(uintptr_t)1023);
  const int STAGES = p.stages, STAGE_BYTES = p.stage_bytes;
  uint64_t* bars = reinterpret_cast<uint64_t*>(smem + PIPE_BYTES + 2 * EPI_BYTES);
  uint64_t* full_bar = bars;
  uint64_t* empty_bar = bars + MAX_STAGES;

  const int wg = __shfl_sync(0xffffffffu, (int)threadIdx.x / 128, 0);
  const int total_tiles = p.tiles_w * p.tiles_h * p.tiles_f * p.n_tiles;
  const bool split = p.nseg > 1;
  const int nplanes = split ? 2 : 1;
  const uint32_t b_bytes = (uint32_t)p.block_n * BLOCK_K * 2;
  const int ksteps = p.ntaps * p.kchunks;

  if (threadIdx.x == 0) {
    asm volatile("prefetch.tensormap [%0];" ::"l"(reinterpret_cast<uint64_t>(&tmap_a)) : "memory");
    asm volatile("prefetch.tensormap [%0];" ::"l"(reinterpret_cast<uint64_t>(&tmap_a2)) : "memory");
    asm volatile("prefetch.tensormap [%0];" ::"l"(reinterpret_cast<uint64_t>(&tmap_b)) : "memory");
    asm volatile("prefetch.tensormap [%0];" ::"l"(reinterpret_cast<uint64_t>(&tmap_o)) : "memory");
    for (int i = 0; i < STAGES; ++i) { mbar_init(&full_bar[i], 1); mbar_init(&empty_bar[i], 1); }
    asm volatile("fence.mbarrier_init.release.cluster;" ::: "memory");
  }
  __syncthreads();

  if (wg == 0) {
    producer_regs();
    if (threadIdx.x == 0) {
      uint32_t stage = 0, phase = 0;
      const uint32_t a_bytes = (uint32_t)(p.bw * p.bh * p.bf) * BLOCK_K * 2;
      const uint32_t tx_bytes = (a_bytes + b_bytes) * nplanes;
      for (int tile = blockIdx.x; tile < total_tiles; tile += gridDim.x) {
        const TileCoord t = decode_tile(p, tile);
        for (int tap = 0; tap < p.ntaps; ++tap) {
          for (int kc = 0; kc < p.kchunks; ++kc) {
            mbar_wait(&empty_bar[stage], phase ^ 1);
            uint8_t* sa = smem + stage * STAGE_BYTES;
            uint8_t* sb = sa + nplanes * A_BYTES;
            mbar_expect_tx(&full_bar[stage], tx_bytes);
            for (int pl = 0; pl < nplanes; ++pl) {
              if (kc < p.kchunks_a1)
                tma_load_4d(sa + pl * A_BYTES, pl ? &tmap_a_lo : &tmap_a, &full_bar[stage], kc * BLOCK_K, t.w0 * p.a_stride + p.tap_dx[tap],
                            t.h0 * p.a_stride + p.tap_dy[tap], t.f0);
              else
                tma_load_4d(sa + pl * A_BYTES, pl ? &tmap_a2_lo : &tmap_a2, &full_bar[stage], (kc - p.kchunks_a1) * BLOCK_K, t.w0 + p.tap_dx[tap],
                            t.h0 + p.tap_dy[tap], t.f0);
              tma_load_3d(sb + pl * b_bytes, pl ? &tmap_b_lo : &tmap_b, &full_bar[stage], kc * BLOCK_K, t.n0, tap);
            }
            if (++stage == STAGES) { stage = 0; phase ^= 1; }
          }
        }
      }
    }
  } else {
    consumer_regs();
    const int cw = wg - 1, row = threadIdx.x & 127;
    const int warp = row / 32, lane = row & 31;
    uint8_t* epi = smem + PIPE_BYTES + cw * EPI_BYTES;
    const float alpha = p.out_f32 ? p.alpha * (p.alpha_dev ? __ldg(p.alpha_dev) : 1.0f) : 1.0f;
    const int my_tiles = (total_tiles - (int)blockIdx.x + (int)gridDim.x - 1) / (int)gridDim.x;
    uint32_t stage = 0, phase = 0;
    if (cw) ring_advance(stage, phase, ksteps, STAGES);
    for (int j = cw; j < my_tiles; j += 2) {
      const TileCoord t = decode_tile(p, (int)blockIdx.x + j * (int)gridDim.x);
      float acc[2][BN / 2];
#pragma unroll
      for (int b = 0; b < 2; ++b)
#pragma unroll
        for (int i = 0; i < BN / 2; ++i) acc[b][i] = 0.f;
      if (j > 0) named_bar_sync(ORDER_BAR + cw, 256);
      uint32_t prev = 0;
      int kc = 0;
      for (int ks = 0; ks < ksteps; ++ks) {
        mbar_wait(&full_bar[stage], phase);
        const uint32_t sa = smem_u32(smem + stage * STAGE_BYTES);
        const uint32_t sb = sa + nplanes * A_BYTES;
        const int kvalid = kc < p.kchunks_a1 ? p.K1 - kc * BLOCK_K : p.K - p.K1 - (kc - p.kchunks_a1) * BLOCK_K;
        const int nk = kvalid >= BLOCK_K ? BLOCK_K / MMA_K : (kvalid + MMA_K - 1) / MMA_K;
        wgmma_fence();
        switch (nk) {
          case 1: mma_stage<BN, 1>(acc[0], acc[1], sa, sb, b_bytes, split); break;
          case 2: mma_stage<BN, 2>(acc[0], acc[1], sa, sb, b_bytes, split); break;
          case 3: mma_stage<BN, 3>(acc[0], acc[1], sa, sb, b_bytes, split); break;
          default: mma_stage<BN, BLOCK_K / MMA_K>(acc[0], acc[1], sa, sb, b_bytes, split); break;
        }
        wgmma_commit();
        wgmma_wait<1>();
        if (ks > 0 && row == 0) mbar_arrive(&empty_bar[prev]);
        prev = stage;
        if (++stage == STAGES) { stage = 0; phase ^= 1; }
        if (++kc == p.kchunks) kc = 0;
      }
      if (j + 1 < my_tiles) named_bar_arrive(ORDER_BAR + (cw ^ 1), 256);
      wgmma_wait<0>();
      if (row == 0) mbar_arrive(&empty_bar[prev]);
      ring_advance(stage, phase, ksteps, STAGES);
      const bool direct = DIRECT && t.f0 >= p.f_direct;
      bool rv[2][2];
      int rpix[2][2];
#pragma unroll
      for (int b = 0; b < 2; ++b)
#pragma unroll
        for (int h = 0; h < 2; ++h) {
          const int r = b * 64 + warp * 16 + (lane >> 2) + 8 * h;
          const int rw = r % p.bw, rh = (r / p.bw) % p.bh, rf = r / (p.bw * p.bh);
          const int w = t.w0 + rw, y = t.h0 + rh, f = t.f0 + rf;
          rv[b][h] = rf < p.bf && w < p.W && y < p.H && f < p.F;
          rpix[b][h] = (f * p.H + y) * p.W + w;
        }
      const int q2 = 2 * (lane & 3);
#pragma unroll
      for (int sl = 0; sl < BN / EPI_COLS; ++sl) {
        const int col = t.n0 + sl * EPI_COLS;
        if (col >= p.Cout) break;
        const bool d1 = col < p.n_split;
        const int cd = d1 ? col : col - p.n_split;
        const int opitch = d1 ? p.out_pitch : p.out2_pitch, ocoff = d1 ? p.out_coff : p.out2_coff;
        float v[2][2][4];
#pragma unroll
        for (int b = 0; b < 2; ++b)
#pragma unroll
          for (int h = 0; h < 2; ++h)
#pragma unroll
            for (int k = 0; k < 2; ++k) {
              const int i = sl * (EPI_COLS / 2) + 4 * k + 2 * h;
              v[b][h][2 * k] = acc[b][i]; v[b][h][2 * k + 1] = acc[b][i + 1];
            }
        const bool planes = p.out_f32 && (d1 ? p.planes : p.planes2);
        if (p.out_f32) {
#pragma unroll
          for (int b = 0; b < 2; ++b)
#pragma unroll
            for (int h = 0; h < 2; ++h)
#pragma unroll
              for (int j = 0; j < 4; ++j) v[b][h][j] = __fmul_rn(v[b][h][j], alpha);
          if (p.bias) {
#pragma unroll
            for (int k = 0; k < 2; ++k) {
              const float2 bb = __ldg(reinterpret_cast<const float2*>(p.bias + col + 8 * k + q2));
#pragma unroll
              for (int b = 0; b < 2; ++b)
#pragma unroll
                for (int h = 0; h < 2; ++h) { v[b][h][2 * k] = __fadd_rn(v[b][h][2 * k], bb.x); v[b][h][2 * k + 1] = __fadd_rn(v[b][h][2 * k + 1], bb.y); }
            }
          }
          if (p.accumulate) {
            const float* o32 = (d1 ? p.out32 : p.out32_2) + ocoff + cd + q2;
#pragma unroll
            for (int b = 0; b < 2; ++b)
#pragma unroll
              for (int h = 0; h < 2; ++h)
                if (rv[b][h])
#pragma unroll
                  for (int k = 0; k < 2; ++k) {
                    const float2 o = *reinterpret_cast<const float2*>(o32 + (long long)rpix[b][h] * opitch + 8 * k);
                    v[b][h][2 * k] = __fadd_rn(v[b][h][2 * k], o.x); v[b][h][2 * k + 1] = __fadd_rn(v[b][h][2 * k + 1], o.y);
                  }
          }
          if (p.relu) {
#pragma unroll
            for (int b = 0; b < 2; ++b)
#pragma unroll
              for (int h = 0; h < 2; ++h)
#pragma unroll
                for (int j = 0; j < 4; ++j) v[b][h][j] = relu(v[b][h][j]);
          }
          if (p.mask32) {
            const float* m32 = p.mask32 + p.mask32_coff + col + q2;
#pragma unroll
            for (int b = 0; b < 2; ++b)
#pragma unroll
              for (int h = 0; h < 2; ++h)
#pragma unroll
                for (int k = 0; k < 2; ++k) {
                  const float2 y = rv[b][h] ? __ldg(reinterpret_cast<const float2*>(m32 + (long long)rpix[b][h] * p.mask32_pitch + 8 * k)) : make_float2(0.f, 0.f);
                  if (!(y.x > 0.f)) v[b][h][2 * k] = 0.f;
                  if (!(y.y > 0.f)) v[b][h][2 * k + 1] = 0.f;
                }
          }
        } else {
          if (p.bias) {
#pragma unroll
            for (int k = 0; k < 2; ++k) {
              const float2 bb = __ldg(reinterpret_cast<const float2*>(p.bias + col + 8 * k + q2));
#pragma unroll
              for (int b = 0; b < 2; ++b)
#pragma unroll
                for (int h = 0; h < 2; ++h) { v[b][h][2 * k] += bb.x; v[b][h][2 * k + 1] += bb.y; }
            }
          }
          if (p.accumulate) {
            const __half* o16 = (d1 ? p.out : p.out2) + ocoff + cd + q2;
#pragma unroll
            for (int b = 0; b < 2; ++b)
#pragma unroll
              for (int h = 0; h < 2; ++h)
                if (rv[b][h])
#pragma unroll
                  for (int k = 0; k < 2; ++k) {
                    const float2 o = __half22float2(*reinterpret_cast<const __half2*>(o16 + (long long)rpix[b][h] * opitch + 8 * k));
                    v[b][h][2 * k] += o.x; v[b][h][2 * k + 1] += o.y;
                  }
          }
          if (p.relu) {
#pragma unroll
            for (int b = 0; b < 2; ++b)
#pragma unroll
              for (int h = 0; h < 2; ++h)
#pragma unroll
                for (int j = 0; j < 4; ++j) v[b][h][j] = relu(v[b][h][j]);
          }
          if (p.mask_y) {
            const __half* my = p.mask_y + p.mask_coff + col + q2;
#pragma unroll
            for (int b = 0; b < 2; ++b)
#pragma unroll
              for (int h = 0; h < 2; ++h)
#pragma unroll
                for (int k = 0; k < 2; ++k) {
                  const float2 y = rv[b][h] ? __half22float2(__ldg(reinterpret_cast<const __half2*>(my + (long long)rpix[b][h] * p.mask_pitch + 8 * k)))
                                            : make_float2(0.f, 0.f);
                  if (!(y.x > 0.f)) v[b][h][2 * k] = 0.f;
                  if (!(y.y > 0.f)) v[b][h][2 * k + 1] = 0.f;
                }
          }
        }
        if (row == 0) bulk_wait_read0();
        named_bar_sync(EPI_BAR + cw, 128);
        const bool scaled = p.flag || p.plane_scale != 1.0f;
        float m = 0.f;
#pragma unroll
        for (int b = 0; b < 2; ++b)
#pragma unroll
          for (int h = 0; h < 2; ++h) {
            const int r = b * 64 + warp * 16 + (lane >> 2) + 8 * h;
            if (p.out_f32) {
              const bool s = (lane >> 3) & 1;
              const float2 x0 = make_float2(v[b][h][0], v[b][h][1]), x1 = make_float2(v[b][h][2], v[b][h][3]);
              *reinterpret_cast<float2*>(epi + sw64_off(r, q2 + (s ? 8 : 0))) = s ? x1 : x0;
              *reinterpret_cast<float2*>(epi + sw64_off(r, q2 + (s ? 0 : 8))) = s ? x0 : x1;
              if (planes)
#pragma unroll
                for (int k = 0; k < 2; ++k) {
                  float x0 = v[b][h][2 * k], x1 = v[b][h][2 * k + 1];
                  if (scaled) {
                    x0 = __fmul_rn(x0, p.plane_scale); x1 = __fmul_rn(x1, p.plane_scale);
                    if (rv[b][h]) {
                      m = fmaxf(m, fabsf(x0)); if (x0 != x0) m = INFINITY;
                      m = fmaxf(m, fabsf(x1)); if (x1 != x1) m = INFINITY;
                    }
                  }
                  const __half2 hh = __floats2half2_rn(x0, x1);
                  const float2 hf = __half22float2(hh);
                  *reinterpret_cast<uint32_t*>(epi + EPI_F32_BYTES + sw32_off(r, 8 * k + q2)) = h2_bits(hh);
                  *reinterpret_cast<uint32_t*>(epi + EPI_F32_BYTES + EPI_F16_BYTES + sw32_off(r, 8 * k + q2)) =
                      h2_bits(__floats2half2_rn(__fsub_rn(x0, hf.x), __fsub_rn(x1, hf.y)));
                }
            } else {
#pragma unroll
              for (int k = 0; k < 2; ++k)
                *reinterpret_cast<uint32_t*>(epi + sw32_off(r, 8 * k + q2)) = h2_bits(__floats2half2_rn(v[b][h][2 * k], v[b][h][2 * k + 1]));
            }
          }
        if (planes && p.flag && !(m <= 65504.f)) *p.flag = 1;
        fence_proxy_async_smem();
        named_bar_sync(EPI_BAR + cw, 128);
        if (row == 0 && !direct) {
          tma_store_4d(d1 ? &tmap_o : &tmap_o2, epi, cd, t.w0, t.h0, t.f0);
          if (planes) {
            tma_store_4d(d1 ? &tmap_o_hi : &tmap_o2_hi, epi + EPI_F32_BYTES, cd, t.w0, t.h0, t.f0);
            tma_store_4d(d1 ? &tmap_o_lo : &tmap_o2_lo, epi + EPI_F32_BYTES + EPI_F16_BYTES, cd, t.w0, t.h0, t.f0);
          }
          bulk_commit();
        }
        if (direct) {
          const int rw = row % p.bw, rh = (row / p.bw) % p.bh, rf = row / (p.bw * p.bh);
          const int w = t.w0 + rw, y = t.h0 + rh, f = t.f0 + rf;
          if (rf < p.bf && w < p.W && y < p.H && f < p.F) {
            const long long po = ((long long)(f * p.H + y) * p.W + w) * opitch + ocoff + cd;
            if (p.out_f32) {
              float* o32 = (d1 ? p.out32 : p.out32_2) + po;
#pragma unroll 1
              for (int j = 0; j < EPI_COLS / 4; ++j)
                *reinterpret_cast<float4*>(o32 + 4 * j) = *reinterpret_cast<const float4*>(epi + sw64_off(row, 4 * j));
            }
            if (!p.out_f32 || planes) {
              const uint8_t* st = epi + (p.out_f32 ? EPI_F32_BYTES : 0);
              char* o16 = reinterpret_cast<char*>((d1 ? p.out : p.out2) + po);
              const long long lo = d1 ? p.out_lo : p.out2_lo;
#pragma unroll 1
              for (int j = 0; j < EPI_COLS / 8; ++j) {
                *reinterpret_cast<uint4*>(o16 + 16 * j) = *reinterpret_cast<const uint4*>(st + sw32_off(row, 8 * j));
                if (planes) *reinterpret_cast<uint4*>(o16 + lo + 16 * j) = *reinterpret_cast<const uint4*>(st + EPI_F16_BYTES + sw32_off(row, 8 * j));
              }
            }
          }
        }
      }
    }
    if (row == 0) bulk_wait0();
  }
}

#define UMMA_CONV_PARAMS                                                                                                    \
  const __grid_constant__ CUtensorMap tmap_a, const __grid_constant__ CUtensorMap tmap_a2, const __grid_constant__ CUtensorMap tmap_b, \
      const __grid_constant__ CUtensorMap tmap_a_lo, const __grid_constant__ CUtensorMap tmap_a2_lo,                               \
      const __grid_constant__ CUtensorMap tmap_b_lo, const __grid_constant__ CUtensorMap tmap_o,                                   \
      const __grid_constant__ CUtensorMap tmap_o_hi, const __grid_constant__ CUtensorMap tmap_o_lo,                                \
      const __grid_constant__ CUtensorMap tmap_o2, const __grid_constant__ CUtensorMap tmap_o2_hi,                                 \
      const __grid_constant__ CUtensorMap tmap_o2_lo, const __grid_constant__ UmmaConvParams p
#define UMMA_CONV_ARGS tmap_a, tmap_a2, tmap_b, tmap_a_lo, tmap_a2_lo, tmap_b_lo, tmap_o, tmap_o_hi, tmap_o_lo, tmap_o2, tmap_o2_hi, tmap_o2_lo, p

template <int BN>
__global__ void __launch_bounds__(NUM_THREADS, 1) umma_conv_kernel(UMMA_CONV_PARAMS) { umma_conv_body<BN, false>(UMMA_CONV_ARGS); }
template <int BN>
__global__ void __launch_bounds__(NUM_THREADS, 1) umma_conv_tail_kernel(UMMA_CONV_PARAMS) { umma_conv_body<BN, true>(UMMA_CONV_ARGS); }

typedef CUresult (*EncodeTiledFn)(CUtensorMap*, CUtensorMapDataType, cuuint32_t, void*, const cuuint64_t*, const cuuint64_t*,
                                  const cuuint32_t*, const cuuint32_t*, CUtensorMapInterleave, CUtensorMapSwizzle,
                                  CUtensorMapL2promotion, CUtensorMapFloatOOBfill);

int resolve_encode(UmmaContext& ctx) {
  if (ctx.encode_tiled) return 0;
  void* fn = nullptr;
  cudaDriverEntryPointQueryResult q;
  cudaError_t e = cudaGetDriverEntryPoint("cuTensorMapEncodeTiled", &fn, cudaEnableDefault, &q);
  if (e != cudaSuccess || q != cudaDriverEntryPointSuccess || !fn) {
    cudaGetLastError();
    set_thread_error("cuTensorMapEncodeTiled not available from the driver");
    return 2;
  }
  ctx.encode_tiled = fn;
  int dev = 0, sms = 132;
  if (cudaGetDevice(&dev) == cudaSuccess) cudaDeviceGetAttribute(&sms, cudaDevAttrMultiProcessorCount, dev);
  ctx.num_sms = sms;
  return 0;
}

int encode(UmmaContext& ctx, CUtensorMap* m, int rank, void* addr, const cuuint64_t* dims, const cuuint64_t* strides,
           const cuuint32_t* box, int spatial_stride = 1, CUtensorMapDataType dtype = CU_TENSOR_MAP_DATA_TYPE_FLOAT16,
           CUtensorMapSwizzle swizzle = CU_TENSOR_MAP_SWIZZLE_128B) {
  cuuint32_t es[5] = {1, (cuuint32_t)spatial_stride, (cuuint32_t)spatial_stride, 1, 1};
  CUresult r = reinterpret_cast<EncodeTiledFn>(ctx.encode_tiled)(m, dtype, (cuuint32_t)rank, addr, dims, strides,
                                                                box, es, CU_TENSOR_MAP_INTERLEAVE_NONE, swizzle,
                                                                CU_TENSOR_MAP_L2_PROMOTION_L2_256B, CU_TENSOR_MAP_FLOAT_OOB_FILL_NONE);
  if (r != CUDA_SUCCESS) {
    char buf[128];
    snprintf(buf, sizeof buf, "cuTensorMapEncodeTiled failed (CUresult %d, rank %d)", (int)r, rank);
    set_thread_error(buf);
    return 2;
  }
  return 0;
}

void pick_box(int W, int& bw, int& bh, int& bf) {
  if (W % 8 == 0 && W >= 56) { bw = 8; bh = 8; bf = 2; }
  else if (W % 4 == 0) { bw = 4; bh = 4; bf = 8; }
  else if (W % 2 == 0) { bw = 2; bh = 2; bf = 32; }
  else if (W <= 8) { bw = W; bh = 1; bf = BLOCK_M / W; }
  else { bw = 1; bh = 1; bf = 128; }
}

int encode_out(UmmaContext& ctx, CUtensorMap* m, const UmmaConvParams& p, const void* base, int pitch, int n, bool f32) {
  const cuuint64_t es = f32 ? 4 : 2;
  cuuint64_t dims[4] = {(cuuint64_t)n, (cuuint64_t)p.W, (cuuint64_t)p.H, (cuuint64_t)p.F};
  cuuint64_t str[3] = {(cuuint64_t)pitch * es, (cuuint64_t)p.W * pitch * es, (cuuint64_t)p.H * p.W * pitch * es};
  cuuint32_t box[4] = {(cuuint32_t)EPI_COLS, (cuuint32_t)p.bw, (cuuint32_t)p.bh, (cuuint32_t)p.bf};
  return encode(ctx, m, 4, const_cast<void*>(base), dims, str, box, 1, f32 ? CU_TENSOR_MAP_DATA_TYPE_FLOAT32 : CU_TENSOR_MAP_DATA_TYPE_FLOAT16,
                f32 ? CU_TENSOR_MAP_SWIZZLE_64B : CU_TENSOR_MAP_SWIZZLE_32B);
}

int encode_planes(UmmaContext& ctx, CUtensorMap* mhi, CUtensorMap* mlo, const UmmaConvParams& p, const __half* hi, long long lo_off, int pitch, int n) {
  if (int rc = encode_out(ctx, mhi, p, hi, pitch, n, false)) return rc;
  return encode_out(ctx, mlo, p, reinterpret_cast<const char*>(hi) + lo_off, pitch, n, false);
}

int bind_out(UmmaContext& ctx, UmmaConvPlan& plan, View o, float* out32, int n, bool second) {
  UmmaConvParams& p = plan.p;
  CUtensorMap* m = second ? &plan.tmap_o2 : &plan.tmap_o;
  CUtensorMap* mhi = second ? &plan.tmap_o2_hi : &plan.tmap_o_hi;
  CUtensorMap* mlo = second ? &plan.tmap_o2_lo : &plan.tmap_o_lo;
  const bool f32 = p.out_f32 != 0;
  if (int rc = encode_out(ctx, m, p, f32 ? (const void*)(out32 + o.coff) : (const void*)(reinterpret_cast<__half*>(o.base) + o.coff), o.pitch, n, f32))
    return rc;
  *mhi = *m; *mlo = *m;
  const int planes = f32 && o.base;
  if (planes)
    if (int rc = encode_planes(ctx, mhi, mlo, p, reinterpret_cast<__half*>(o.base) + o.coff, o.lo_off, o.pitch, n)) return rc;
  (second ? p.planes2 : p.planes) = planes;
  (second ? p.out2_lo : p.out_lo) = planes ? o.lo_off : 0;
  return 0;
}

int bind_common(UmmaContext& ctx, UmmaConvPlan& plan, View a, View o, int F, int K, int N, int ntaps, const __half* w,
                int a_stride = 1, const UmmaTcOpts* tc = nullptr) {
  plan.enabled = false;
  if (int rc = resolve_encode(ctx)) return rc;
  if (a_stride == 2 || (a_stride == 1 && (a.H != o.H || a.W != o.W))) {
    View ao = a; ao.H = o.H; ao.W = o.W;
    if (int rc = bind_common(ctx, plan, ao, o, F, K, N, ntaps, w, 1, tc)) return rc;
    plan.enabled = false;
    UmmaConvParams& q = plan.p;
    q.a_stride = a_stride;
    cuuint64_t dims[4] = {(cuuint64_t)K, (cuuint64_t)a.W, (cuuint64_t)a.H, (cuuint64_t)F};
    cuuint64_t str[3] = {(cuuint64_t)a.pitch * 2, (cuuint64_t)a.W * a.pitch * 2, (cuuint64_t)a.H * a.W * a.pitch * 2};
    cuuint32_t box[4] = {(cuuint32_t)BLOCK_K, (cuuint32_t)(a_stride * q.bw), (cuuint32_t)(a_stride * q.bh), (cuuint32_t)q.bf};
    if (int rc = encode(ctx, &plan.tmap_a, 4, reinterpret_cast<__half*>(a.base) + a.coff, dims, str, box, a_stride)) return rc;
    plan.tmap_a_lo = plan.tmap_a;
    if (a.lo_off)
      if (int rc = encode(ctx, &plan.tmap_a_lo, 4, reinterpret_cast<__half*>(reinterpret_cast<char*>(a.base) + a.lo_off) + a.coff, dims, str, box, a_stride))
        return rc;
    plan.tmap_a2 = plan.tmap_a; plan.tmap_a2_lo = plan.tmap_a_lo;
    plan.enabled = true;
    return 0;
  }
  if (a.H != o.H || a.W != o.W) { set_thread_error("umma conv: geometry mismatch"); return 1; }
  if (K % 8 || N % 16 || a.pitch % 8 || a.coff % 8 || o.pitch % 8 || o.coff % 8 || ntaps > UMMA_MAX_TAPS) {
    set_thread_error("umma conv: unsupported channel alignment"); return 1; }
  UmmaConvParams& p = plan.p;
  memset(&p, 0, sizeof(p));
  p.W = a.W; p.H = a.H; p.F = F; p.f_direct = 1 << 30;
  pick_box(a.W, p.bw, p.bh, p.bf);
  p.tiles_w = (a.W + p.bw - 1) / p.bw; p.tiles_h = (a.H + p.bh - 1) / p.bh; p.tiles_f = (F + p.bf - 1) / p.bf;
  p.n_tiles = (N + MAX_BLOCK_N - 1) / MAX_BLOCK_N;
  p.block_n = (((N + p.n_tiles - 1) / p.n_tiles) + N_STEP - 1) / N_STEP * N_STEP;
  p.kchunks = (K + BLOCK_K - 1) / BLOCK_K;
  p.K = K;
  p.ntaps = ntaps;
  p.out = reinterpret_cast<__half*>(o.base); p.out_pitch = o.pitch; p.out_coff = o.coff; p.Cout = N;
  p.a_stride = 1; p.mask_y = nullptr; p.mask_pitch = 0; p.mask_coff = 0;
  p.kchunks_a1 = (K + BLOCK_K - 1) / BLOCK_K; p.K1 = K; p.n_split = 1 << 30; p.out2 = p.out; p.out2_pitch = o.pitch; p.out2_coff = o.coff;
  {
    cuuint64_t dims[4] = {(cuuint64_t)K, (cuuint64_t)a.W, (cuuint64_t)a.H, (cuuint64_t)F};
    cuuint64_t str[3] = {(cuuint64_t)a.pitch * 2, (cuuint64_t)a.W * a.pitch * 2, (cuuint64_t)a.H * a.W * a.pitch * 2};
    cuuint32_t box[4] = {(cuuint32_t)BLOCK_K, (cuuint32_t)p.bw, (cuuint32_t)p.bh, (cuuint32_t)p.bf};
    if (int rc = encode(ctx, &plan.tmap_a, 4, reinterpret_cast<__half*>(a.base) + a.coff, dims, str, box)) return rc;
    plan.tmap_a_lo = plan.tmap_a;
    if (a.lo_off)
      if (int rc = encode(ctx, &plan.tmap_a_lo, 4, reinterpret_cast<__half*>(reinterpret_cast<char*>(a.base) + a.lo_off) + a.coff, dims, str, box)) return rc;
  }
  {
    cuuint64_t dims[3] = {(cuuint64_t)K, (cuuint64_t)N, (cuuint64_t)ntaps};
    cuuint64_t str[2] = {(cuuint64_t)K * 2, (cuuint64_t)N * K * 2};
    cuuint32_t box[3] = {(cuuint32_t)BLOCK_K, (cuuint32_t)p.block_n, 1};
    if (int rc = encode(ctx, &plan.tmap_b, 3, const_cast<__half*>(w), dims, str, box)) return rc;
    plan.b_lo_off = tc ? tc->w_lo_off : 0;
    plan.tmap_b_lo = plan.tmap_b;
    if (plan.b_lo_off)
      if (int rc = encode(ctx, &plan.tmap_b_lo, 3, reinterpret_cast<__half*>(reinterpret_cast<char*>(const_cast<__half*>(w)) + plan.b_lo_off), dims, str, box)) return rc;
  }
  plan.tmap_a2 = plan.tmap_a; plan.tmap_a2_lo = plan.tmap_a_lo;
  p.nseg = tc ? 3 : 1; p.out_f32 = tc ? 1 : 0;
  p.stage_bytes = ((A_BYTES + p.block_n * BLOCK_K * 2) * (tc ? 2 : 1) + 1023) / 1024 * 1024;
  p.stages = PIPE_BYTES / p.stage_bytes; if (p.stages > MAX_STAGES) p.stages = MAX_STAGES;
  p.alpha = tc ? tc->alpha : 1.0f; p.alpha_dev = tc ? tc->alpha_dev : nullptr;
  p.mask32 = nullptr; p.mask32_pitch = 0; p.mask32_coff = 0; p.plane_scale = 1.0f; p.flag = nullptr;
  p.out32 = tc ? tc->out32 : nullptr;
  if (tc && (!tc->out32 || !a.lo_off || !tc->w_lo_off)) { set_thread_error("umma conv: split-operand bind needs operand planes and an fp32 output"); return 1; }
  if (int rc = bind_out(ctx, plan, o, p.out32, N, false)) return rc;
  p.out32_2 = p.out32; p.planes2 = p.planes; p.out2_lo = p.out_lo;
  plan.tmap_o2 = plan.tmap_o; plan.tmap_o2_hi = plan.tmap_o_hi; plan.tmap_o2_lo = plan.tmap_o_lo;
  plan.enabled = true;
  return 0;
}

void mark_tc_ok(UmmaConvPlan& plan, int W, bool two_sources) {
  UmmaConvParams& p = plan.p;
  p.tc_ok = 0;
  if (!plan.enabled || p.a_stride != 1) return;
  if (!(p.ntaps == 1 || p.ntaps == 4 || p.ntaps == 9)) return;
  if (p.kchunks_a1 != p.kchunks && (p.ntaps != 1 || !two_sources)) return;
  if (p.out_pitch % 16 || p.out_coff % 16 || p.out2_pitch % 16 || p.out2_coff % 16 || p.n_split % 16 || (p.bias && p.n_tiles * p.block_n > 1024)) return;
  if (W < 7) return;
  p.tc_ok = 1;
}

}

int umma_resolve_encode(UmmaContext& ctx) { return resolve_encode(ctx); }
int umma_encode_f16(UmmaContext& ctx, CUtensorMap* m, int rank, void* addr, const cuuint64_t* dims,
                    const cuuint64_t* strides, const cuuint32_t* box, int spatial_stride) {
  return encode(ctx, m, rank, addr, dims, strides, box, spatial_stride);
}

void umma_context_init(UmmaContext&) {}
void umma_context_destroy(UmmaContext&) {}

int umma_conv_bind_taps(UmmaContext& ctx, UmmaConvPlan& plan, View in, View out, int F, int cin, int cout, int ntaps,
                        const int* dy, const int* dx, const __half* w_tap_n_k, const float* bias, int relu, const UmmaTcOpts* tc, int stride) {
  if (stride != 1 && stride != 2) { set_thread_error("umma conv: stride must be 1 or 2"); return 1; }
  if (int rc = bind_common(ctx, plan, in, out, F, cin, cout, ntaps, w_tap_n_k, stride, tc)) return rc;
  for (int t = 0; t < ntaps; ++t) { plan.p.tap_dy[t] = dy[t]; plan.p.tap_dx[t] = dx[t]; }
  plan.p.bias = bias; plan.p.relu = relu; plan.p.accumulate = 0;
  mark_tc_ok(plan, in.W, false);
  return 0;
}

int umma_conv_bind_fwd(UmmaContext& ctx, UmmaConvPlan& plan, View in, View out, int F, int cin, int cout, int k, int pad,
                       int stride, const __half* w_tap_n_k, const float* bias, const UmmaTcOpts* tc) {
  if (stride != 1 && stride != 2) { set_thread_error("umma conv: stride must be 1 or 2"); return 1; }
  if (int rc = bind_common(ctx, plan, in, out, F, cin, cout, k * k, w_tap_n_k, stride, tc)) return rc;
  for (int r = 0; r < k; ++r)
    for (int s = 0; s < k; ++s) { plan.p.tap_dy[r * k + s] = r - pad; plan.p.tap_dx[r * k + s] = s - pad; }
  plan.p.bias = bias; plan.p.relu = 1; plan.p.accumulate = 0;
  mark_tc_ok(plan, in.W, false);
  return 0;
}

int umma_conv_bind_dgrad(UmmaContext& ctx, UmmaConvPlan& plan, View dz, View dx, int F, int cin, int cout, int k, int pad,
                         const __half* w_tap_k_n, int accumulate, const UmmaTcOpts* tc) {
  if (int rc = bind_common(ctx, plan, dz, dx, F, cout, cin, k * k, w_tap_k_n, 1, tc)) return rc;
  for (int r = 0; r < k; ++r)
    for (int s = 0; s < k; ++s) { plan.p.tap_dy[r * k + s] = pad - r; plan.p.tap_dx[r * k + s] = pad - s; }
  plan.p.bias = nullptr; plan.p.relu = 0; plan.p.accumulate = accumulate;
  mark_tc_ok(plan, dz.W, false);
  return 0;
}

int umma_conv_bind_fused_fwd(UmmaContext& ctx, UmmaConvPlan& plan, View in, View out1, View out2, int F, int cin, int n1, int n2,
                             const __half* w_n_k, const float* bias, const UmmaTcOpts* tc) {
  View o = out1; o.C = n1 + n2;
  if (out1.H != out2.H || out1.W != out2.W || n1 % 16 || n2 % 16 || out2.pitch % 8 || out2.coff % 8) { set_thread_error("fused fwd: bad views"); return 1; }
  if (tc && !tc->out32_2) { set_thread_error("fused fwd: the split-operand bind needs both fp32 destinations"); return 1; }
  if (int rc = bind_common(ctx, plan, in, o, F, cin, n1 + n2, 1, w_n_k, 1, tc)) return rc;
  plan.p.tap_dy[0] = 0; plan.p.tap_dx[0] = 0;
  plan.p.bias = bias; plan.p.relu = 1; plan.p.accumulate = 0;
  plan.p.n_split = n1; plan.p.out2 = reinterpret_cast<__half*>(out2.base); plan.p.out2_pitch = out2.pitch; plan.p.out2_coff = out2.coff;
  if (tc) plan.p.out32_2 = tc->out32_2;
  if (int rc = bind_out(ctx, plan, out1, plan.p.out32, n1, false)) { plan.enabled = false; return rc; }
  if (int rc = bind_out(ctx, plan, out2, plan.p.out32_2, n2, true)) { plan.enabled = false; return rc; }
  mark_tc_ok(plan, in.W, false);
  return 0;
}

int umma_conv_bind_fused_dgrad(UmmaContext& ctx, UmmaConvPlan& plan, View dz1, View dz2, View dx, int F, int cin, int k1, int k2,
                               const __half* w_n_k, int accumulate, const UmmaTcOpts* tc) {
  const int k1p = (k1 + BLOCK_K - 1) / BLOCK_K * BLOCK_K;
  View a = k1 ? dz1 : dz2;
  if (int rc = bind_common(ctx, plan, a, dx, F, k1 ? k1 : k2, cin, 1, w_n_k, 1, tc)) return rc;
  UmmaConvParams& p = plan.p;
  p.tap_dy[0] = 0; p.tap_dx[0] = 0; p.bias = nullptr; p.relu = 0; p.accumulate = accumulate;
  if (k1) {
    if (dz2.H != dz1.H || dz2.W != dz1.W || dz2.pitch % 8 || dz2.coff % 8 || k2 % 8) { set_thread_error("fused dgrad: bad views"); return 1; }
    cuuint64_t dims[4] = {(cuuint64_t)k2, (cuuint64_t)dz2.W, (cuuint64_t)dz2.H, (cuuint64_t)F};
    cuuint64_t str[3] = {(cuuint64_t)dz2.pitch * 2, (cuuint64_t)dz2.W * dz2.pitch * 2, (cuuint64_t)dz2.H * dz2.W * dz2.pitch * 2};
    cuuint32_t box[4] = {(cuuint32_t)BLOCK_K, (cuuint32_t)p.bw, (cuuint32_t)p.bh, (cuuint32_t)p.bf};
    if (int rc = encode(ctx, &plan.tmap_a2, 4, reinterpret_cast<__half*>(dz2.base) + dz2.coff, dims, str, box)) { plan.enabled = false; return rc; }
    p.kchunks_a1 = k1p / BLOCK_K; p.K1 = k1; p.K = k1 + k2;
    p.kchunks = p.kchunks_a1 + (k2 + BLOCK_K - 1) / BLOCK_K;
    cuuint64_t bd[3] = {(cuuint64_t)(k1p + k2), (cuuint64_t)cin, 1};
    cuuint64_t bs[2] = {(cuuint64_t)(k1p + k2) * 2, (cuuint64_t)cin * (k1p + k2) * 2};
    cuuint32_t bb[3] = {(cuuint32_t)BLOCK_K, (cuuint32_t)p.block_n, 1};
    if (int rc = encode(ctx, &plan.tmap_b, 3, const_cast<__half*>(w_n_k), bd, bs, bb)) { plan.enabled = false; return rc; }
    plan.tmap_b_lo = plan.tmap_b;
    if (plan.b_lo_off)
      if (int rc = encode(ctx, &plan.tmap_b_lo, 3, reinterpret_cast<__half*>(reinterpret_cast<char*>(const_cast<__half*>(w_n_k)) + plan.b_lo_off), bd, bs, bb)) {
        plan.enabled = false; return rc; }
    if (tc && !dz2.lo_off) { set_thread_error("fused dgrad: the split-operand bind needs the second source's operand planes"); plan.enabled = false; return 1; }
    plan.tmap_a2_lo = plan.tmap_a2;
    if (dz2.lo_off)
      if (int rc = encode(ctx, &plan.tmap_a2_lo, 4, reinterpret_cast<__half*>(reinterpret_cast<char*>(dz2.base) + dz2.lo_off) + dz2.coff, dims, str, box)) {
        plan.enabled = false; return rc; }
  }
  mark_tc_ok(plan, a.W, k1 != 0);
  return 0;
}

void umma_conv_set_mask(UmmaConvPlan& plan, View y) {
  plan.mask_y = reinterpret_cast<const __half*>(y.base); plan.mask_pitch = y.pitch; plan.mask_coff = y.coff;
}

int umma_conv_set_mask_tc(UmmaContext& ctx, UmmaConvPlan& plan, View y32, View dplanes, float plane_scale, int* flag) {
  if (int rc = encode_planes(ctx, &plan.tmap_mask_hi, &plan.tmap_mask_lo, plan.p, reinterpret_cast<__half*>(dplanes.base) + dplanes.coff, dplanes.lo_off,
                             dplanes.pitch, plan.p.Cout)) return rc;
  plan.mask32 = reinterpret_cast<const float*>(y32.base); plan.mask32_pitch = y32.pitch; plan.mask32_coff = y32.coff;
  plan.mask_planes = true; plan.mask_plane_scale = plane_scale; plan.mask_flag = flag;
  return 0;
}

namespace {
template <int BN, bool DIRECT>
int launch_bn(const UmmaConvPlan& plan, const UmmaConvParams& p, const CUtensorMap& o_hi, const CUtensorMap& o_lo, int grid, cudaStream_t s) {
  static bool attr_set[64] = {};
  auto kern = DIRECT ? umma_conv_tail_kernel<BN> : umma_conv_kernel<BN>;
  int dev = 0;
  cudaGetDevice(&dev);
  if (dev < 0 || dev >= 64 || !attr_set[dev]) {
    if (cudaFuncSetAttribute(kern, cudaFuncAttributeMaxDynamicSharedMemorySize, SMEM_BYTES) != cudaSuccess) {
      set_thread_error("umma conv: cannot raise dynamic shared memory limit"); cudaGetLastError(); return 2; }
    if (dev >= 0 && dev < 64) attr_set[dev] = true;
  }
  kern<<<grid, NUM_THREADS, SMEM_BYTES, s>>>(plan.tmap_a, plan.tmap_a2, plan.tmap_b, plan.tmap_a_lo, plan.tmap_a2_lo, plan.tmap_b_lo, plan.tmap_o, o_hi, o_lo,
                                             plan.tmap_o2, plan.tmap_o2_hi, plan.tmap_o2_lo, p);
  SSNB_LAUNCH_CHECK("umma_conv_kernel");
  return 0;
}
template <int BN>
int launch_bn(const UmmaConvPlan& plan, const UmmaConvParams& p, const CUtensorMap& o_hi, const CUtensorMap& o_lo, int grid, cudaStream_t s) {
  return p.f_direct < (1 << 30) ? launch_bn<BN, true>(plan, p, o_hi, o_lo, grid, s) : launch_bn<BN, false>(plan, p, o_hi, o_lo, grid, s);
}
}

int umma_conv_launch(UmmaContext& ctx, const UmmaConvPlan& plan, cudaStream_t s, bool mask, int frames) {
  if (!plan.enabled) { set_thread_error("umma conv: plan not bound"); return 3; }
  UmmaConvParams p = plan.p;
  if (frames && frames != p.F) {
    if (frames < 1 || frames > p.F || mask || p.accumulate) { set_thread_error("umma conv: a frame count below the plan's runs forward plans only"); return 3; }
    p.F = frames;
    p.tiles_f = (frames + p.bf - 1) / p.bf;
    if (frames % p.bf) p.f_direct = frames - frames % p.bf;
  }
  if (mask && plan.mask_y) { p.mask_y = plan.mask_y; p.mask_pitch = plan.mask_pitch; p.mask_coff = plan.mask_coff; }
  const bool mplanes = mask && p.out_f32 && plan.mask32 && plan.mask_planes;
  if (mplanes) {
    p.mask32 = plan.mask32; p.mask32_pitch = plan.mask32_pitch; p.mask32_coff = plan.mask32_coff;
    p.planes = 1; p.plane_scale = plan.mask_plane_scale; p.flag = plan.mask_flag;
  }
  if (p.out_f32 && p.mask_y) { set_thread_error("umma conv: the fp32 epilogue takes its mask through mask32"); return 3; }
  const CUtensorMap& o_hi = mplanes ? plan.tmap_mask_hi : plan.tmap_o_hi;
  const CUtensorMap& o_lo = mplanes ? plan.tmap_mask_lo : plan.tmap_o_lo;
  const int total = p.tiles_w * p.tiles_h * p.tiles_f * p.n_tiles;
  const int grid = total < ctx.num_sms ? total : ctx.num_sms;
  t_tag.tiles = total; t_tag.block_n = p.block_n;
  switch (p.block_n) {
    case 16: return launch_bn<16>(plan, p, o_hi, o_lo, grid, s);
    case 32: return launch_bn<32>(plan, p, o_hi, o_lo, grid, s);
    case 48: return launch_bn<48>(plan, p, o_hi, o_lo, grid, s);
    case 64: return launch_bn<64>(plan, p, o_hi, o_lo, grid, s);
    case 80: return launch_bn<80>(plan, p, o_hi, o_lo, grid, s);
    case 96: return launch_bn<96>(plan, p, o_hi, o_lo, grid, s);
    case 112: return launch_bn<112>(plan, p, o_hi, o_lo, grid, s);
    case 128: return launch_bn<128>(plan, p, o_hi, o_lo, grid, s);
  }
  set_thread_error("umma conv: unsupported tile width"); return 3;
}

}
```

### action-detection_b200/csrc/umma_conv.cuh

```cuda
#pragma once
#include <cuda.h>
#include <cuda_fp16.h>
#include <cuda_runtime.h>

#include "common.cuh"

namespace ssnb {

constexpr int UMMA_MAX_TAPS = 25;

struct UmmaContext {
  void* encode_tiled = nullptr;
  int num_sms = 132;
};

struct UmmaConvParams {
  int W, H, F;
  int bw, bh, bf;
  int tiles_w, tiles_h, tiles_f;
  int f_direct;
  long long out_lo, out2_lo;
  int n_tiles, block_n;
  int stages, stage_bytes;
  int kchunks, ntaps, K;
  int tap_dy[UMMA_MAX_TAPS], tap_dx[UMMA_MAX_TAPS];
  __half* out; int out_pitch, out_coff, Cout;
  int a_stride;
  const float* bias;
  int relu, accumulate;
  int kchunks_a1, K1;
  int n_split;
  __half* out2; int out2_pitch, out2_coff;
  int tc_ok;
  const __half* mask_y; int mask_pitch, mask_coff;
  int nseg, out_f32;
  float alpha;
  const float* alpha_dev;
  float* out32; int planes;
  float* out32_2; int planes2;
  const float* mask32; int mask32_pitch, mask32_coff;
  float plane_scale; int* flag;
};

struct UmmaConvPlan {
  bool enabled = false;
  const __half* mask_y = nullptr; int mask_pitch = 0, mask_coff = 0;
  CUtensorMap tmap_a, tmap_a2, tmap_b;
  CUtensorMap tmap_a_lo, tmap_a2_lo, tmap_b_lo;
  long long b_lo_off = 0;
  CUtensorMap tmap_o, tmap_o_hi, tmap_o_lo, tmap_o2, tmap_o2_hi, tmap_o2_lo;
  const float* mask32 = nullptr; int mask32_pitch = 0, mask32_coff = 0;
  CUtensorMap tmap_mask_hi, tmap_mask_lo; bool mask_planes = false; float mask_plane_scale = 1.0f; int* mask_flag = nullptr;
  UmmaConvParams p;
};

struct UmmaTcOpts { long long w_lo_off = 0; float* out32 = nullptr; float alpha = 1.0f; const float* alpha_dev = nullptr; float* out32_2 = nullptr; };
void umma_context_init(UmmaContext& ctx);
void umma_context_destroy(UmmaContext& ctx);
int umma_conv_bind_fwd(UmmaContext& ctx, UmmaConvPlan& plan, View in, View out, int F, int cin, int cout, int k, int pad,
                       int stride, const __half* w_tap_n_k, const float* bias, const UmmaTcOpts* tc = nullptr);
int umma_conv_bind_taps(UmmaContext& ctx, UmmaConvPlan& plan, View in, View out, int F, int cin, int cout, int ntaps,
                        const int* dy, const int* dx, const __half* w_tap_n_k, const float* bias, int relu, const UmmaTcOpts* tc = nullptr,
                        int stride = 1);
int umma_conv_bind_dgrad(UmmaContext& ctx, UmmaConvPlan& plan, View dz, View dx, int F, int cin, int cout, int k, int pad,
                         const __half* w_tap_k_n, int accumulate, const UmmaTcOpts* tc = nullptr);
int umma_conv_bind_fused_fwd(UmmaContext& ctx, UmmaConvPlan& plan, View in, View out1, View out2, int F, int cin, int n1, int n2,
                             const __half* w_n_k, const float* bias, const UmmaTcOpts* tc = nullptr);
int umma_conv_bind_fused_dgrad(UmmaContext& ctx, UmmaConvPlan& plan, View dz1, View dz2, View dx, int F, int cin, int k1, int k2,
                               const __half* w_n_k, int accumulate, const UmmaTcOpts* tc = nullptr);
int umma_conv_launch(UmmaContext& ctx, const UmmaConvPlan& plan, cudaStream_t s, bool mask = false, int frames = 0);
void umma_conv_set_mask(UmmaConvPlan& plan, View y);
int umma_conv_set_mask_tc(UmmaContext& ctx, UmmaConvPlan& plan, View y32, View dplanes, float plane_scale, int* flag);

int umma_resolve_encode(UmmaContext& ctx);
int umma_encode_f16(UmmaContext& ctx, CUtensorMap* m, int rank, void* addr, const cuuint64_t* dims,
                    const cuuint64_t* strides, const cuuint32_t* box, int spatial_stride = 1);

struct UmmaWgradParams {
  int W, H, F;
  int bw, bh, bf;
  int tiles_w, tiles_h, tiles_f;
  int ptiles_per_split, splits;
  int ntaps, tap_dy[UMMA_MAX_TAPS], tap_dx[UMMA_MAX_TAPS];
  int Cout, Cin, m_tiles, n_tiles, block_n;
  int x_stride;
  float* bias_partial;
  int taps_per_cta, tap_groups;
  int stages, stage_bytes;
  float* partial;
  int nseg;
  int sub_dh, sub_df;
};
struct UmmaWgradPlan {
  bool enabled = false;
  CUtensorMap tmap_dz, tmap_x;
  CUtensorMap tmap_dz_lo, tmap_x_lo;
  UmmaWgradParams p;
};
constexpr int UMMA_WGRAD_MAX_PTILES = 768;
int umma_wgrad_ptiles(int W, int H, int F);
int umma_wgrad_splits(int ctas, int ptiles, int num_sms, int waves = 1);
int umma_wgrad_bind(UmmaContext& ctx, UmmaWgradPlan& plan, View dz, View x, int F, int cin, int cout, int k, int pad,
                    float* partial, int max_splits, int x_stride = 1);
int umma_wgrad_bind_taps(UmmaContext& ctx, UmmaWgradPlan& plan, View dz, View x, int F, int cin, int cout, int ntaps,
                         const int* dy, const int* dx, float* partial, int max_splits, int x_stride = 1);
int umma_wgrad_launch(UmmaContext& ctx, const UmmaWgradPlan& plan, cudaStream_t s, float* bias_partial = nullptr);

}
```

Before: 821.0.

## Compute stride-2 conv data gradient by output phase instead of zero-upsampling

Stride-2 convolution backward data no longer materialises a zero-interleaved upsampled gradient buffer before running a stride-1 conv. Instead, each tap is mapped to one of four output phases and loads a compact half-size gradient tile into one smem slot, zero-filled elsewhere. Only the wgmma pass for that phase's accumulator half is issued, and the output is stored through per-phase strided tensor maps. This removes the upsample kernel, its memory traffic, and the MMAs spent on zeros, at the cost of extra tensor maps, a larger kernel parameter block and more complex epilogue indexing.

Result: slower. 790.9, median of 6 (-3.7%).

```diff
diff --git a/action-detection_b200/csrc/common.cuh b/action-detection_b200/csrc/common.cuh
--- a/action-detection_b200/csrc/common.cuh
+++ b/action-detection_b200/csrc/common.cuh
@@ -148,6 +148,5 @@
 int launch_pack_conv1_s2d(const __half* wd, int Cout, int Cin, int Cs, __half* ws, cudaStream_t s);
 int launch_wgrad_finalize_s2d(const float* partial, int splits, int Cout, int Cin, int Cs, const float* mult, float out_scale,
                               const float* unscale, float* dw_ref, int accumulate, cudaStream_t s);
-int launch_upsample2_zero(View src, __half* dst, int H, int W, int F, cudaStream_t s);
 
 }
diff --git a/action-detection_b200/csrc/engine.cu b/action-detection_b200/csrc/engine.cu
--- a/action-detection_b200/csrc/engine.cu
+++ b/action-detection_b200/csrc/engine.cu
@@ -108,7 +108,7 @@
 
 struct ssnb_engine : ssnb::Graph<ssnb::Op> {
   ssnb_config cfg;
-  size_t up_plane = 0, s2d_plane = 0, s2d_w_plane = 0;
+  size_t s2d_plane = 0, s2d_w_plane = 0;
   int* tc_flag = nullptr;
   size_t tc_flag_off = 0;
   float* gscale = nullptr;
@@ -118,7 +118,7 @@
   size_t bn_stat_off = 0, bn_partial_off = 0;
   std::vector<FusedBlock> fused;
   size_t ws_bytes = 0, partial_off = 0, partial_bytes = 0, bpartial_off = 0;
-  size_t s2d_off = 0, s2d_w_off = 0, up_off = 0;
+  size_t s2d_off = 0, s2d_w_off = 0;
   bool fold_pools = true;
   bool s2d_ready = false;
   int Cs = 0;
@@ -319,13 +319,13 @@
     e->s2d_off = operand_region(F * 112 * 112 * 4 * e->Cs * 2, e->s2d_plane);
     e->s2d_w_off = operand_region((size_t)16 * 64 * e->Cs * 2, e->s2d_w_plane);
     if (e->cfg.training) {
-      size_t up = 0;
+      size_t unused = 0, plane = 0;
       for (const Op& o : e->ops)
         if (o.kind == OP_CONV && o.stride == 2 && o.conv != 0) {
           const Buffer& ib = e->bufs[e->vals[o.in].buf];
-          up = std::max(up, F * ib.H * ib.W * (size_t)e->convs[o.conv].cout * 2);
+          unused = std::max(unused, F * ib.H * ib.W * (size_t)e->convs[o.conv].cout * 2);
         }
-      e->up_off = operand_region(up, e->up_plane);
+      operand_region(unused, plane);
       pmax = std::max(pmax, (size_t)e->conv1_tsplits * 16 * 64 * e->Cs * 4);
     }
   }
@@ -440,7 +440,7 @@
                     launch_avgpool3_vec<__half>(dout, din, View(), F, o.grad_accumulate, s));
   }
   const Conv& c = e->convs[o.conv];
-  const View x = e->view(o.in, false), y = e->view(o.out, false), dy = e->view(o.out, true);
+  const View y = e->view(o.out, false), dy = e->view(o.out, true);
   const float* scale = (const float*)(e->ws + e->packed[o.conv].scale);
   float* bpartial = (float*)(e->ws + e->bpartial_off);
   float* dbp = (e->db.size() && e->db[o.conv]) ? e->db[o.conv] : nullptr;
@@ -476,11 +476,6 @@
     }
   }
   if (rc) return rc;
-  if (tc_x && c.stride == 2 && o.conv != 0) {
-    View dz = e->operand(o.out, true);
-    for (int p = 0; p < e->nplanes(); ++p, dz.base = (char*)dz.base + dz.lo_off)
-      if ((rc = launch_upsample2_zero(dz, (__half*)(e->ws + e->up_off + p * e->up_plane), x.H, x.W, F, s))) return rc;
-  }
   if (tc_w) {
     float* partial = (float*)(e->ws + o.partial_off);
     float* bp = bias_w ? (float*)(e->ws + o.bias_partial_off) : nullptr;
@@ -608,13 +603,11 @@
                             c.stride, h->w_fwd(pk), (const float*)(h->ws + pk.bias), h->tc_opts(tf, pk.wplane, h->view(o.out, false).base, 1.0f, pk.wmax));
     if (rc) return h->fail(rc, "bind_fwd(" + c.id + "): " + ssnb::thread_error());
     if (!training) continue;
-    const View in = h->view(o.in, false);
-    View dz = h->operand(o.out, true);
-    if (c.stride == 2) { dz.base = h->ws + h->up_off; dz.H = in.H; dz.W = in.W; dz.C = c.cout; dz.pitch = c.cout; dz.coff = 0; dz.lo_off = (long long)h->up_plane; }
     View dx = h->view(o.in, true);
     const UmmaTcOpts* og = h->tc_opts(tg, pk.wplane, dx.base, 1.0f / gs, pk.wmax);
     if (og) dx.base = nullptr;
-    rc = umma_conv_bind_dgrad(h->umma_ctx, o.umma_dgrad, dz, dx, h->F, c.cin, c.cout, c.kh, c.ph, h->w_dgrad(pk), o.grad_accumulate, og);
+    rc = umma_conv_bind_dgrad(h->umma_ctx, o.umma_dgrad, h->operand(o.out, true), dx, h->F, c.cin, c.cout, c.kh, c.ph, h->w_dgrad(pk),
+                              o.grad_accumulate, og, c.stride);
     if (rc) return h->fail(rc, "bind_dgrad(" + c.id + "): " + ssnb::thread_error());
     tc_gate(o.umma_dgrad);
     if (use_wgrad && (rc = umma_wgrad_bind(h->umma_ctx, o.umma_wgrad, h->operand(o.out, true), h->operand(o.in, false), h->F, c.cin, c.cout,
diff --git a/action-detection_b200/csrc/s2d_glue.cu b/action-detection_b200/csrc/s2d_glue.cu
--- a/action-detection_b200/csrc/s2d_glue.cu
+++ b/action-detection_b200/csrc/s2d_glue.cu
@@ -113,24 +113,6 @@
   }
 }
 
-__global__ void upsample2_zero_kernel(const __half* __restrict__ src, int OH, int OW, int C, int spitch, int scoff,
-                                      __half* __restrict__ dst, int H, int W, int F) {
-  const int G = C / 8;
-  const long long total = (long long)F * H * W * G;
-  const long long i = (long long)blockIdx.x * blockDim.x + threadIdx.x;
-  if (i >= total) return;
-  const unsigned iu = (unsigned)i;
-  const int g = (int)(iu % (unsigned)G);
-  const unsigned pu = iu / (unsigned)G;
-  const int x = (int)(pu % (unsigned)W), y = (int)((pu / (unsigned)W) % (unsigned)H);
-  const long long p = pu;
-  const long long f = pu / (unsigned)(W * H);
-  uint4 v = make_uint4(0u, 0u, 0u, 0u);
-  if (!(x & 1) && !(y & 1) && y / 2 < OH && x / 2 < OW)
-    v = __ldg(reinterpret_cast<const uint4*>(src + ((f * OH + y / 2) * OW + x / 2) * spitch + scoff + g * 8));
-  *reinterpret_cast<uint4*>(dst + p * C + g * 8) = v;
-}
-
 }
 
 int launch_nhwc_to_s2d(View src, int F, __half* dst, long long lo_off, int Cs, cudaStream_t s) {
@@ -169,11 +151,5 @@
   SSNB_LAUNCH_CHECK("wgrad_finalize_s2d_kernel");
   return 0;
 }
-int launch_upsample2_zero(View src, __half* dst, int H, int W, int F, cudaStream_t s) {
-  const long long n = (long long)F * H * W * (src.C / 8);
-  upsample2_zero_kernel<<<(unsigned)((n + 255) / 256), 256, 0, s>>>((const __half*)src.base, src.H, src.W, src.C, src.pitch, src.coff, dst, H, W, F);
-  SSNB_LAUNCH_CHECK("upsample2_zero_kernel");
-  return 0;
-}
 
 }
diff --git a/action-detection_b200/csrc/umma_conv.cu b/action-detection_b200/csrc/umma_conv.cu
--- a/action-detection_b200/csrc/umma_conv.cu
+++ b/action-detection_b200/csrc/umma_conv.cu
@@ -27,6 +27,9 @@
 constexpr int EPI_BAR = 3;
 static_assert(SMEM_BYTES <= 227 * 1024, "shared memory per block");
 
+constexpr int SLOT_ROWS = 32;
+constexpr int SLOT_BYTES = SLOT_ROWS * BLOCK_K * 2;
+
 struct TileCoord { int w0, h0, f0, n0; };
 __device__ __forceinline__ TileCoord decode_tile(const UmmaConvParams& p, int tile) {
   TileCoord t;
@@ -63,6 +66,25 @@
   mma_k<BN, NK>(d0, d1, sa, sb);
 }
 
+template <int BN, int NK>
+__device__ __forceinline__ void mma_half(float* d, uint32_t sa, uint32_t sb, uint32_t b_bytes, bool split) {
+#pragma unroll
+  for (int pass = split ? 0 : 2; pass < 3; ++pass) {
+    const uint32_t a = sa + (pass == 0 ? A_BYTES : 0), b = sb + (pass == 1 ? b_bytes : 0);
+#pragma unroll
+    for (int k = 0; k < NK; ++k) wgmma<BN, 0, 0>(d, make_desc_sw128(a + k * MMA_K * 2), make_desc_sw128(b + k * MMA_K * 2));
+  }
+}
+template <int BN>
+__device__ __forceinline__ void mma_half_nk(float* d, int nk, uint32_t sa, uint32_t sb, uint32_t b_bytes, bool split) {
+  switch (nk) {
+    case 1: mma_half<BN, 1>(d, sa, sb, b_bytes, split); break;
+    case 2: mma_half<BN, 2>(d, sa, sb, b_bytes, split); break;
+    case 3: mma_half<BN, 3>(d, sa, sb, b_bytes, split); break;
+    default: mma_half<BN, BLOCK_K / MMA_K>(d, sa, sb, b_bytes, split); break;
+  }
+}
+
 __device__ __forceinline__ void ring_advance(uint32_t& stage, uint32_t& phase, int n, int stages) {
   const uint32_t s = stage + (uint32_t)n;
   phase ^= (s / (uint32_t)stages) & 1u;
@@ -74,7 +96,7 @@
 umma_conv_body(const CUtensorMap& tmap_a, const CUtensorMap& tmap_a2, const CUtensorMap& tmap_b, const CUtensorMap& tmap_a_lo,
                const CUtensorMap& tmap_a2_lo, const CUtensorMap& tmap_b_lo, const CUtensorMap& tmap_o, const CUtensorMap& tmap_o_hi,
                const CUtensorMap& tmap_o_lo, const CUtensorMap& tmap_o2, const CUtensorMap& tmap_o2_hi, const CUtensorMap& tmap_o2_lo,
-               const UmmaConvParams& p) {
+               const UmmaPhaseMaps& pm, const UmmaConvParams& p) {
   extern __shared__ uint8_t smem_raw[];
   uint8_t* smem = reinterpret_cast<uint8_t*>((reinterpret_cast<uintptr_t>(smem_raw) + 1023) & ~(uintptr_t)1023);
   const int STAGES = p.stages, STAGE_BYTES = p.stage_bytes;
@@ -88,7 +110,16 @@
   const int nplanes = split ? 2 : 1;
   const uint32_t b_bytes = (uint32_t)p.block_n * BLOCK_K * 2;
   const int ksteps = p.ntaps * p.kchunks;
-
+  const int os = DIRECT ? 1 : p.ostride;
+
+  if (os == 2) {
+    for (int i = threadIdx.x; i < STAGES * nplanes * 2 * (SLOT_BYTES / 16); i += blockDim.x) {
+      const int c = i % (SLOT_BYTES / 16), part = (i / (SLOT_BYTES / 16)) & 1, sp = i / (SLOT_BYTES / 16) / 2;
+      *reinterpret_cast<uint4*>(smem + (sp / nplanes) * STAGE_BYTES + (sp % nplanes) * A_BYTES + part * 2 * SLOT_BYTES + c * 16) =
+          make_uint4(0u, 0u, 0u, 0u);
+    }
+    fence_proxy_async_smem();
+  }
   if (threadIdx.x == 0) {
     asm volatile("prefetch.tensormap [%0];" ::"l"(reinterpret_cast<uint64_t>(&tmap_a)) : "memory");
     asm volatile("prefetch.tensormap [%0];" ::"l"(reinterpret_cast<uint64_t>(&tmap_a2)) : "memory");
@@ -103,7 +134,7 @@
     producer_regs();
     if (threadIdx.x == 0) {
       uint32_t stage = 0, phase = 0;
-      const uint32_t a_bytes = (uint32_t)(p.bw * p.bh * p.bf) * BLOCK_K * 2;
+      const uint32_t a_bytes = os == 2 ? (uint32_t)SLOT_BYTES : (uint32_t)(p.bw * p.bh * p.bf) * BLOCK_K * 2;
       const uint32_t tx_bytes = (a_bytes + b_bytes) * nplanes;
       for (int tile = blockIdx.x; tile < total_tiles; tile += gridDim.x) {
         const TileCoord t = decode_tile(p, tile);
@@ -114,7 +145,10 @@
             uint8_t* sb = sa + nplanes * A_BYTES;
             mbar_expect_tx(&full_bar[stage], tx_bytes);
             for (int pl = 0; pl < nplanes; ++pl) {
-              if (kc < p.kchunks_a1)
+              if (os == 2)
+                tma_load_4d(sa + pl * A_BYTES + SLOT_BYTES, pl ? &tmap_a_lo : &tmap_a, &full_bar[stage], kc * BLOCK_K, t.w0 / 2 + p.tap_dx[tap],
+                            t.h0 / 2 + p.tap_dy[tap], t.f0);
+              else if (kc < p.kchunks_a1)
                 tma_load_4d(sa + pl * A_BYTES, pl ? &tmap_a_lo : &tmap_a, &full_bar[stage], kc * BLOCK_K, t.w0 * p.a_stride + p.tap_dx[tap],
                             t.h0 * p.a_stride + p.tap_dy[tap], t.f0);
               else
@@ -145,7 +179,7 @@
         for (int i = 0; i < BN / 2; ++i) acc[b][i] = 0.f;
       if (j > 0) named_bar_sync(ORDER_BAR + cw, 256);
       uint32_t prev = 0;
-      int kc = 0;
+      int kc = 0, tap = 0;
       for (int ks = 0; ks < ksteps; ++ks) {
         mbar_wait(&full_bar[stage], phase);
         const uint32_t sa = smem_u32(smem + stage * STAGE_BYTES);
@@ -153,18 +187,25 @@
         const int kvalid = kc < p.kchunks_a1 ? p.K1 - kc * BLOCK_K : p.K - p.K1 - (kc - p.kchunks_a1) * BLOCK_K;
         const int nk = kvalid >= BLOCK_K ? BLOCK_K / MMA_K : (kvalid + MMA_K - 1) / MMA_K;
         wgmma_fence();
-        switch (nk) {
-          case 1: mma_stage<BN, 1>(acc[0], acc[1], sa, sb, b_bytes, split); break;
-          case 2: mma_stage<BN, 2>(acc[0], acc[1], sa, sb, b_bytes, split); break;
-          case 3: mma_stage<BN, 3>(acc[0], acc[1], sa, sb, b_bytes, split); break;
-          default: mma_stage<BN, BLOCK_K / MMA_K>(acc[0], acc[1], sa, sb, b_bytes, split); break;
+        if (os == 2) {
+          const int q = p.tap_ph[tap];
+          const uint32_t ha = sa + ((q & 1) ? 0u : (uint32_t)SLOT_BYTES);
+          if (q >> 1) mma_half_nk<BN>(acc[1], nk, ha, sb, b_bytes, split);
+          else mma_half_nk<BN>(acc[0], nk, ha, sb, b_bytes, split);
+        } else {
+          switch (nk) {
+            case 1: mma_stage<BN, 1>(acc[0], acc[1], sa, sb, b_bytes, split); break;
+            case 2: mma_stage<BN, 2>(acc[0], acc[1], sa, sb, b_bytes, split); break;
+            case 3: mma_stage<BN, 3>(acc[0], acc[1], sa, sb, b_bytes, split); break;
+            default: mma_stage<BN, BLOCK_K / MMA_K>(acc[0], acc[1], sa, sb, b_bytes, split); break;
+          }
         }
         wgmma_commit();
         wgmma_wait<1>();
         if (ks > 0 && row == 0) mbar_arrive(&empty_bar[prev]);
         prev = stage;
         if (++stage == STAGES) { stage = 0; phase ^= 1; }
-        if (++kc == p.kchunks) kc = 0;
+        if (++kc == p.kchunks) { kc = 0; ++tap; }
       }
       if (j + 1 < my_tiles) named_bar_arrive(ORDER_BAR + (cw ^ 1), 256);
       wgmma_wait<0>();
@@ -173,13 +214,15 @@
       const bool direct = DIRECT && t.f0 >= p.f_direct;
       bool rv[2][2];
       int rpix[2][2];
+      const int sbw = p.bw / os, sbh = p.bh / os;
 #pragma unroll
       for (int b = 0; b < 2; ++b)
 #pragma unroll
         for (int h = 0; h < 2; ++h) {
           const int r = b * 64 + warp * 16 + (lane >> 2) + 8 * h;
-          const int rw = r % p.bw, rh = (r / p.bw) % p.bh, rf = r / (p.bw * p.bh);
-          const int w = t.w0 + rw, y = t.h0 + rh, f = t.f0 + rf;
+          const int q = os == 2 ? r / SLOT_ROWS : 0, i = os == 2 ? r % SLOT_ROWS : r;
+          const int rw = i % sbw, rh = (i / sbw) % sbh, rf = i / (sbw * sbh);
+          const int w = (t.w0 / os + rw) * os + (q & 1), y = (t.h0 / os + rh) * os + (q >> 1), f = t.f0 + rf;
           rv[b][h] = rf < p.bf && w < p.W && y < p.H && f < p.F;
           rpix[b][h] = (f * p.H + y) * p.W + w;
         }
@@ -341,10 +384,22 @@
         fence_proxy_async_smem();
         named_bar_sync(EPI_BAR + cw, 128);
         if (row == 0 && !direct) {
-          tma_store_4d(d1 ? &tmap_o : &tmap_o2, epi, cd, t.w0, t.h0, t.f0);
-          if (planes) {
-            tma_store_4d(d1 ? &tmap_o_hi : &tmap_o2_hi, epi + EPI_F32_BYTES, cd, t.w0, t.h0, t.f0);
-            tma_store_4d(d1 ? &tmap_o_lo : &tmap_o2_lo, epi + EPI_F32_BYTES + EPI_F16_BYTES, cd, t.w0, t.h0, t.f0);
+          if (os == 2) {
+            const int rb = p.out_f32 ? 64 : 32;
+            for (int q = 0; q < 4; ++q) {
+              tma_store_4d(q ? &pm.o[q - 1] : &tmap_o, epi + q * SLOT_ROWS * rb, cd, t.w0 / 2, t.h0 / 2, t.f0);
+              if (planes) {
+                tma_store_4d(q ? &pm.hi[q - 1] : &tmap_o_hi, epi + EPI_F32_BYTES + q * SLOT_ROWS * 32, cd, t.w0 / 2, t.h0 / 2, t.f0);
+                tma_store_4d(q ? &pm.lo[q - 1] : &tmap_o_lo, epi + EPI_F32_BYTES + EPI_F16_BYTES + q * SLOT_ROWS * 32, cd, t.w0 / 2,
+                             t.h0 / 2, t.f0);
+              }
+            }
+          } else {
+            tma_store_4d(d1 ? &tmap_o : &tmap_o2, epi, cd, t.w0, t.h0, t.f0);
+            if (planes) {
+              tma_store_4d(d1 ? &tmap_o_hi : &tmap_o2_hi, epi + EPI_F32_BYTES, cd, t.w0, t.h0, t.f0);
+              tma_store_4d(d1 ? &tmap_o_lo : &tmap_o2_lo, epi + EPI_F32_BYTES + EPI_F16_BYTES, cd, t.w0, t.h0, t.f0);
+            }
           }
           bulk_commit();
         }
@@ -383,8 +438,10 @@
       const __grid_constant__ CUtensorMap tmap_b_lo, const __grid_constant__ CUtensorMap tmap_o,                                   \
       const __grid_constant__ CUtensorMap tmap_o_hi, const __grid_constant__ CUtensorMap tmap_o_lo,                                \
       const __grid_constant__ CUtensorMap tmap_o2, const __grid_constant__ CUtensorMap tmap_o2_hi,                                 \
-      const __grid_constant__ CUtensorMap tmap_o2_lo, const __grid_constant__ UmmaConvParams p
-#define UMMA_CONV_ARGS tmap_a, tmap_a2, tmap_b, tmap_a_lo, tmap_a2_lo, tmap_b_lo, tmap_o, tmap_o_hi, tmap_o_lo, tmap_o2, tmap_o2_hi, tmap_o2_lo, p
+      const __grid_constant__ CUtensorMap tmap_o2_lo, const __grid_constant__ UmmaPhaseMaps pm,                                    \
+      const __grid_constant__ UmmaConvParams p
+#define UMMA_CONV_ARGS tmap_a, tmap_a2, tmap_b, tmap_a_lo, tmap_a2_lo, tmap_b_lo, tmap_o, tmap_o_hi, tmap_o_lo, tmap_o2, tmap_o2_hi, tmap_o2_lo, pm, p
+static_assert(12 * sizeof(CUtensorMap) + sizeof(UmmaPhaseMaps) + sizeof(UmmaConvParams) <= 4096, "kernel parameter size");
 
 template <int BN>
 __global__ void __launch_bounds__(NUM_THREADS, 1) umma_conv_kernel(UMMA_CONV_PARAMS) { umma_conv_body<BN, false>(UMMA_CONV_ARGS); }
@@ -436,32 +493,37 @@
   else { bw = 1; bh = 1; bf = 128; }
 }
 
-int encode_out(UmmaContext& ctx, CUtensorMap* m, const UmmaConvParams& p, const void* base, int pitch, int n, bool f32) {
-  const cuuint64_t es = f32 ? 4 : 2;
-  cuuint64_t dims[4] = {(cuuint64_t)n, (cuuint64_t)p.W, (cuuint64_t)p.H, (cuuint64_t)p.F};
-  cuuint64_t str[3] = {(cuuint64_t)pitch * es, (cuuint64_t)p.W * pitch * es, (cuuint64_t)p.H * p.W * pitch * es};
-  cuuint32_t box[4] = {(cuuint32_t)EPI_COLS, (cuuint32_t)p.bw, (cuuint32_t)p.bh, (cuuint32_t)p.bf};
-  return encode(ctx, m, 4, const_cast<void*>(base), dims, str, box, 1, f32 ? CU_TENSOR_MAP_DATA_TYPE_FLOAT32 : CU_TENSOR_MAP_DATA_TYPE_FLOAT16,
+int encode_out(UmmaContext& ctx, CUtensorMap* m, const UmmaConvParams& p, const void* base, int pitch, int n, bool f32, int q = 0) {
+  const cuuint64_t es = f32 ? 4 : 2, os = (cuuint64_t)p.ostride, W = p.W, H = p.H;
+  cuuint64_t dims[4] = {(cuuint64_t)n, W / os, H / os, (cuuint64_t)p.F};
+  cuuint64_t str[3] = {os * pitch * es, os * W * pitch * es, H * W * pitch * es};
+  cuuint32_t box[4] = {(cuuint32_t)EPI_COLS, (cuuint32_t)(p.bw / os), (cuuint32_t)(p.bh / os), (cuuint32_t)p.bf};
+  const char* at = reinterpret_cast<const char*>(base) + ((long long)(q / 2) * W + q % 2) * pitch * es;
+  return encode(ctx, m, 4, const_cast<char*>(at), dims, str, box, 1, f32 ? CU_TENSOR_MAP_DATA_TYPE_FLOAT32 : CU_TENSOR_MAP_DATA_TYPE_FLOAT16,
                 f32 ? CU_TENSOR_MAP_SWIZZLE_64B : CU_TENSOR_MAP_SWIZZLE_32B);
 }
 
-int encode_planes(UmmaContext& ctx, CUtensorMap* mhi, CUtensorMap* mlo, const UmmaConvParams& p, const __half* hi, long long lo_off, int pitch, int n) {
-  if (int rc = encode_out(ctx, mhi, p, hi, pitch, n, false)) return rc;
-  return encode_out(ctx, mlo, p, reinterpret_cast<const char*>(hi) + lo_off, pitch, n, false);
+int encode_planes(UmmaContext& ctx, CUtensorMap* mhi, CUtensorMap* mlo, const UmmaConvParams& p, const __half* hi, long long lo_off, int pitch, int n,
+                  int q = 0) {
+  if (int rc = encode_out(ctx, mhi, p, hi, pitch, n, false, q)) return rc;
+  return encode_out(ctx, mlo, p, reinterpret_cast<const char*>(hi) + lo_off, pitch, n, false, q);
 }
 
 int bind_out(UmmaContext& ctx, UmmaConvPlan& plan, View o, float* out32, int n, bool second) {
   UmmaConvParams& p = plan.p;
-  CUtensorMap* m = second ? &plan.tmap_o2 : &plan.tmap_o;
-  CUtensorMap* mhi = second ? &plan.tmap_o2_hi : &plan.tmap_o_hi;
-  CUtensorMap* mlo = second ? &plan.tmap_o2_lo : &plan.tmap_o_lo;
   const bool f32 = p.out_f32 != 0;
-  if (int rc = encode_out(ctx, m, p, f32 ? (const void*)(out32 + o.coff) : (const void*)(reinterpret_cast<__half*>(o.base) + o.coff), o.pitch, n, f32))
-    return rc;
-  *mhi = *m; *mlo = *m;
   const int planes = f32 && o.base;
-  if (planes)
-    if (int rc = encode_planes(ctx, mhi, mlo, p, reinterpret_cast<__half*>(o.base) + o.coff, o.lo_off, o.pitch, n)) return rc;
+  for (int q = 0; q < (second ? 1 : p.ostride * p.ostride); ++q) {
+    CUtensorMap* m = second ? &plan.tmap_o2 : q ? &plan.ph.o[q - 1] : &plan.tmap_o;
+    CUtensorMap* mhi = second ? &plan.tmap_o2_hi : q ? &plan.ph.hi[q - 1] : &plan.tmap_o_hi;
+    CUtensorMap* mlo = second ? &plan.tmap_o2_lo : q ? &plan.ph.lo[q - 1] : &plan.tmap_o_lo;
+    if (int rc = encode_out(ctx, m, p, f32 ? (const void*)(out32 + o.coff) : (const void*)(reinterpret_cast<__half*>(o.base) + o.coff), o.pitch, n,
+                            f32, q))
+      return rc;
+    *mhi = *m; *mlo = *m;
+    if (planes)
+      if (int rc = encode_planes(ctx, mhi, mlo, p, reinterpret_cast<__half*>(o.base) + o.coff, o.lo_off, o.pitch, n, q)) return rc;
+  }
   (second ? p.planes2 : p.planes) = planes;
   (second ? p.out2_lo : p.out_lo) = planes ? o.lo_off : 0;
   return 0;
@@ -502,6 +564,8 @@
   p.kchunks = (K + BLOCK_K - 1) / BLOCK_K;
   p.K = K;
   p.ntaps = ntaps;
+  p.ostride = 1;
+  plan.ph = plan.ph_mask = UmmaPhaseMaps{};
   p.out = reinterpret_cast<__half*>(o.base); p.out_pitch = o.pitch; p.out_coff = o.coff; p.Cout = N;
   p.a_stride = 1; p.mask_y = nullptr; p.mask_pitch = 0; p.mask_coff = 0;
   p.kchunks_a1 = (K + BLOCK_K - 1) / BLOCK_K; p.K1 = K; p.n_split = 1 << 30; p.out2 = p.out; p.out2_pitch = o.pitch; p.out2_coff = o.coff;
@@ -583,12 +647,39 @@
 }
 
 int umma_conv_bind_dgrad(UmmaContext& ctx, UmmaConvPlan& plan, View dz, View dx, int F, int cin, int cout, int k, int pad,
-                         const __half* w_tap_k_n, int accumulate, const UmmaTcOpts* tc) {
+                         const __half* w_tap_k_n, int accumulate, const UmmaTcOpts* tc, int stride) {
+  if (stride == 1) {
+    if (int rc = bind_common(ctx, plan, dz, dx, F, cout, cin, k * k, w_tap_k_n, 1, tc)) return rc;
+    for (int r = 0; r < k; ++r)
+      for (int s = 0; s < k; ++s) { plan.p.tap_dy[r * k + s] = pad - r; plan.p.tap_dx[r * k + s] = pad - s; }
+    plan.p.bias = nullptr; plan.p.relu = 0; plan.p.accumulate = accumulate;
+    mark_tc_ok(plan, dz.W, false);
+    return 0;
+  }
+  if (stride != 2 || k * k > UMMA_MAX_TAPS || dx.H % 2 || dx.W % 2) {
+    set_thread_error("umma conv: a phase-split data gradient needs stride 2, k <= 5 and an even output size"); return 1; }
   if (int rc = bind_common(ctx, plan, dz, dx, F, cout, cin, k * k, w_tap_k_n, 1, tc)) return rc;
+  UmmaConvParams& p = plan.p;
+  plan.enabled = false;
+  p.bias = nullptr; p.relu = 0; p.accumulate = accumulate;
+  p.ostride = 2;
   for (int r = 0; r < k; ++r)
-    for (int s = 0; s < k; ++s) { plan.p.tap_dy[r * k + s] = pad - r; plan.p.tap_dx[r * k + s] = pad - s; }
-  plan.p.bias = nullptr; plan.p.relu = 0; plan.p.accumulate = accumulate;
-  mark_tc_ok(plan, dz.W, false);
+    for (int s = 0; s < k; ++s) {
+      const int py = (r - pad) & 1, px = (s - pad) & 1;
+      p.tap_dy[r * k + s] = (py + pad - r) / 2; p.tap_dx[r * k + s] = (px + pad - s) / 2; p.tap_ph[r * k + s] = 2 * py + px;
+    }
+  cuuint64_t dims[4] = {(cuuint64_t)cout, (cuuint64_t)dz.W, (cuuint64_t)dz.H, (cuuint64_t)F};
+  cuuint64_t str[3] = {(cuuint64_t)dz.pitch * 2, (cuuint64_t)dz.W * dz.pitch * 2, (cuuint64_t)dz.H * dz.W * dz.pitch * 2};
+  cuuint32_t box[4] = {(cuuint32_t)BLOCK_K, (cuuint32_t)(p.bw / 2), (cuuint32_t)(p.bh / 2), (cuuint32_t)p.bf};
+  if (int rc = encode(ctx, &plan.tmap_a, 4, reinterpret_cast<__half*>(dz.base) + dz.coff, dims, str, box)) return rc;
+  plan.tmap_a_lo = plan.tmap_a;
+  if (dz.lo_off)
+    if (int rc = encode(ctx, &plan.tmap_a_lo, 4, reinterpret_cast<__half*>(reinterpret_cast<char*>(dz.base) + dz.lo_off) + dz.coff, dims, str, box))
+      return rc;
+  plan.tmap_a2 = plan.tmap_a; plan.tmap_a2_lo = plan.tmap_a_lo;
+  if (int rc = bind_out(ctx, plan, dx, p.out32, cin, false)) return rc;
+  plan.enabled = true;
+  mark_tc_ok(plan, dx.W, false);
   return 0;
 }
 
@@ -646,8 +737,12 @@
 }
 
 int umma_conv_set_mask_tc(UmmaContext& ctx, UmmaConvPlan& plan, View y32, View dplanes, float plane_scale, int* flag) {
-  if (int rc = encode_planes(ctx, &plan.tmap_mask_hi, &plan.tmap_mask_lo, plan.p, reinterpret_cast<__half*>(dplanes.base) + dplanes.coff, dplanes.lo_off,
-                             dplanes.pitch, plan.p.Cout)) return rc;
+  for (int q = 0; q < 3; ++q) plan.ph_mask.o[q] = plan.ph.o[q];
+  for (int q = 0; q < plan.p.ostride * plan.p.ostride; ++q) {
+    if (int rc = encode_planes(ctx, q ? &plan.ph_mask.hi[q - 1] : &plan.tmap_mask_hi, q ? &plan.ph_mask.lo[q - 1] : &plan.tmap_mask_lo, plan.p,
+                               reinterpret_cast<__half*>(dplanes.base) + dplanes.coff, dplanes.lo_off, dplanes.pitch, plan.p.Cout, q))
+      return rc;
+  }
   plan.mask32 = reinterpret_cast<const float*>(y32.base); plan.mask32_pitch = y32.pitch; plan.mask32_coff = y32.coff;
   plan.mask_planes = true; plan.mask_plane_scale = plane_scale; plan.mask_flag = flag;
   return 0;
@@ -655,7 +750,8 @@
 
 namespace {
 template <int BN, bool DIRECT>
-int launch_bn(const UmmaConvPlan& plan, const UmmaConvParams& p, const CUtensorMap& o_hi, const CUtensorMap& o_lo, int grid, cudaStream_t s) {
+int launch_bn(const UmmaConvPlan& plan, const UmmaConvParams& p, const CUtensorMap& o_hi, const CUtensorMap& o_lo, const UmmaPhaseMaps& pm, int grid,
+              cudaStream_t s) {
   static bool attr_set[64] = {};
   auto kern = DIRECT ? umma_conv_tail_kernel<BN> : umma_conv_kernel<BN>;
   int dev = 0;
@@ -666,13 +762,14 @@
     if (dev >= 0 && dev < 64) attr_set[dev] = true;
   }
   kern<<<grid, NUM_THREADS, SMEM_BYTES, s>>>(plan.tmap_a, plan.tmap_a2, plan.tmap_b, plan.tmap_a_lo, plan.tmap_a2_lo, plan.tmap_b_lo, plan.tmap_o, o_hi, o_lo,
-                                             plan.tmap_o2, plan.tmap_o2_hi, plan.tmap_o2_lo, p);
+                                             plan.tmap_o2, plan.tmap_o2_hi, plan.tmap_o2_lo, pm, p);
   SSNB_LAUNCH_CHECK("umma_conv_kernel");
   return 0;
 }
 template <int BN>
-int launch_bn(const UmmaConvPlan& plan, const UmmaConvParams& p, const CUtensorMap& o_hi, const CUtensorMap& o_lo, int grid, cudaStream_t s) {
-  return p.f_direct < (1 << 30) ? launch_bn<BN, true>(plan, p, o_hi, o_lo, grid, s) : launch_bn<BN, false>(plan, p, o_hi, o_lo, grid, s);
+int launch_bn(const UmmaConvPlan& plan, const UmmaConvParams& p, const CUtensorMap& o_hi, const CUtensorMap& o_lo, const UmmaPhaseMaps& pm, int grid,
+              cudaStream_t s) {
+  return p.f_direct < (1 << 30) ? launch_bn<BN, true>(plan, p, o_hi, o_lo, pm, grid, s) : launch_bn<BN, false>(plan, p, o_hi, o_lo, pm, grid, s);
 }
 }
 
@@ -680,7 +777,8 @@
   if (!plan.enabled) { set_thread_error("umma conv: plan not bound"); return 3; }
   UmmaConvParams p = plan.p;
   if (frames && frames != p.F) {
-    if (frames < 1 || frames > p.F || mask || p.accumulate) { set_thread_error("umma conv: a frame count below the plan's runs forward plans only"); return 3; }
+    if (frames < 1 || frames > p.F || mask || p.accumulate || p.ostride > 1) {
+      set_thread_error("umma conv: a frame count below the plan's runs forward plans only"); return 3; }
     p.F = frames;
     p.tiles_f = (frames + p.bf - 1) / p.bf;
     if (frames % p.bf) p.f_direct = frames - frames % p.bf;
@@ -694,18 +792,19 @@
   if (p.out_f32 && p.mask_y) { set_thread_error("umma conv: the fp32 epilogue takes its mask through mask32"); return 3; }
   const CUtensorMap& o_hi = mplanes ? plan.tmap_mask_hi : plan.tmap_o_hi;
   const CUtensorMap& o_lo = mplanes ? plan.tmap_mask_lo : plan.tmap_o_lo;
+  const UmmaPhaseMaps& pm = mplanes ? plan.ph_mask : plan.ph;
   const int total = p.tiles_w * p.tiles_h * p.tiles_f * p.n_tiles;
   const int grid = total < ctx.num_sms ? total : ctx.num_sms;
   t_tag.tiles = total; t_tag.block_n = p.block_n;
   switch (p.block_n) {
-    case 16: return launch_bn<16>(plan, p, o_hi, o_lo, grid, s);
-    case 32: return launch_bn<32>(plan, p, o_hi, o_lo, grid, s);
-    case 48: return launch_bn<48>(plan, p, o_hi, o_lo, grid, s);
-    case 64: return launch_bn<64>(plan, p, o_hi, o_lo, grid, s);
-    case 80: return launch_bn<80>(plan, p, o_hi, o_lo, grid, s);
-    case 96: return launch_bn<96>(plan, p, o_hi, o_lo, grid, s);
-    case 112: return launch_bn<112>(plan, p, o_hi, o_lo, grid, s);
-    case 128: return launch_bn<128>(plan, p, o_hi, o_lo, grid, s);
+    case 16: return launch_bn<16>(plan, p, o_hi, o_lo, pm, grid, s);
+    case 32: return launch_bn<32>(plan, p, o_hi, o_lo, pm, grid, s);
+    case 48: return launch_bn<48>(plan, p, o_hi, o_lo, pm, grid, s);
+    case 64: return launch_bn<64>(plan, p, o_hi, o_lo, pm, grid, s);
+    case 80: return launch_bn<80>(plan, p, o_hi, o_lo, pm, grid, s);
+    case 96: return launch_bn<96>(plan, p, o_hi, o_lo, pm, grid, s);
+    case 112: return launch_bn<112>(plan, p, o_hi, o_lo, pm, grid, s);
+    case 128: return launch_bn<128>(plan, p, o_hi, o_lo, pm, grid, s);
   }
   set_thread_error("umma conv: unsupported tile width"); return 3;
 }
diff --git a/action-detection_b200/csrc/umma_conv.cuh b/action-detection_b200/csrc/umma_conv.cuh
--- a/action-detection_b200/csrc/umma_conv.cuh
+++ b/action-detection_b200/csrc/umma_conv.cuh
@@ -24,6 +24,8 @@
   int stages, stage_bytes;
   int kchunks, ntaps, K;
   int tap_dy[UMMA_MAX_TAPS], tap_dx[UMMA_MAX_TAPS];
+  int ostride;
+  int tap_ph[UMMA_MAX_TAPS];
   __half* out; int out_pitch, out_coff, Cout;
   int a_stride;
   const float* bias;
@@ -42,6 +44,8 @@
   float plane_scale; int* flag;
 };
 
+struct UmmaPhaseMaps { CUtensorMap o[3], hi[3], lo[3]; };
+
 struct UmmaConvPlan {
   bool enabled = false;
   const __half* mask_y = nullptr; int mask_pitch = 0, mask_coff = 0;
@@ -51,6 +55,7 @@
   CUtensorMap tmap_o, tmap_o_hi, tmap_o_lo, tmap_o2, tmap_o2_hi, tmap_o2_lo;
   const float* mask32 = nullptr; int mask32_pitch = 0, mask32_coff = 0;
   CUtensorMap tmap_mask_hi, tmap_mask_lo; bool mask_planes = false; float mask_plane_scale = 1.0f; int* mask_flag = nullptr;
+  UmmaPhaseMaps ph, ph_mask;
   UmmaConvParams p;
 };
 
@@ -63,7 +68,7 @@
                         const int* dy, const int* dx, const __half* w_tap_n_k, const float* bias, int relu, const UmmaTcOpts* tc = nullptr,
                         int stride = 1);
 int umma_conv_bind_dgrad(UmmaContext& ctx, UmmaConvPlan& plan, View dz, View dx, int F, int cin, int cout, int k, int pad,
-                         const __half* w_tap_k_n, int accumulate, const UmmaTcOpts* tc = nullptr);
+                         const __half* w_tap_k_n, int accumulate, const UmmaTcOpts* tc = nullptr, int stride = 1);
 int umma_conv_bind_fused_fwd(UmmaContext& ctx, UmmaConvPlan& plan, View in, View out1, View out2, int F, int cin, int n1, int n2,
                              const __half* w_n_k, const float* bias, const UmmaTcOpts* tc = nullptr);
 int umma_conv_bind_fused_dgrad(UmmaContext& ctx, UmmaConvPlan& plan, View dz1, View dz2, View dx, int F, int cin, int k1, int k2,
```
